# druskus20/volym

Hardware: AMD Instinct MI355X
Metric: Mrays/s + achieved HBM GB/s, 256^3 uint8 @ 1920x1080 (higher is better)
Workload: dtype u8 voxels, f32 compositing

## Files before the change

include/volym_hip.h:

```cpp
#ifndef VOLYM_HIP_H
#define VOLYM_HIP_H

#include <stddef.h>
#include <stdint.h>

#ifdef __cplusplus
extern "C" {
#endif

#define VOLYM_ABI_VERSION 2

enum {
    VOLYM_OK = 0,
    VOLYM_E_INVALID = -1,
    VOLYM_E_HIP = -2,
    VOLYM_E_NO_DEVICE = -3,
    VOLYM_E_NOMEM = -4,
    VOLYM_E_STATE = -5
};

enum { VOLYM_FILTER_NEAREST = 0, VOLYM_FILTER_LINEAR = 1 };

enum {
    VOLYM_OPT_KERNEL = 1,
// ... 9 lines not shown
    VOLYM_OPT_SETUP_IEEE = 10
};

typedef struct volym_camera_uniforms {
    float view_matrix[4][4];
    float projection_matrix[4][4];
    float inverse_view_proj[4][4];
    float camera_position[3];
    float _padding;
} volym_camera_uniforms;

typedef struct volym_parameter_uniforms {
    float density_threshold;
    uint32_t use_cone_importance_check;
    uint32_t use_importance_coloring;
    uint32_t use_opacity;
    uint32_t use_importance_rendering;
    uint32_t use_gaussian_smoothing;
    uint32_t importance_check_ahead_steps;
    float raymarching_step_size;
} volym_parameter_uniforms;

typedef struct volym_stats {
    uint64_t n_vol;
    uint64_t n_imp;
    uint64_t n_steps;
    uint64_t n_dense;
    uint64_t n_hit;
    uint64_t n_rays;
} volym_stats;

typedef struct volym_ctx volym_ctx;

int volym_create(volym_ctx** out, uint32_t width, uint32_t height, int device_id);
void volym_destroy(volym_ctx* ctx);
const char* volym_last_error(const volym_ctx* ctx);
int volym_abi_version(void);

int volym_set_stream(volym_ctx* ctx, void* hip_stream);
int volym_set_option(volym_ctx* ctx, int key, int value);

int volym_set_shard(volym_ctx* ctx, uint32_t rank, uint32_t world);

int volym_set_volume(volym_ctx* ctx, const uint8_t* voxels, uint32_t nx, uint32_t ny,
                     uint32_t nz, int filter);
int volym_set_importances(volym_ctx* ctx, const uint8_t* importances, uint32_t nx,
                          uint32_t ny, uint32_t nz);
int volym_set_labels(volym_ctx* ctx, const uint8_t* labels, uint32_t nx, uint32_t ny, uint32_t nz);
int volym_set_segment_importances(volym_ctx* ctx, const uint8_t table[256]);
int volym_label_counts(volym_ctx* ctx, uint64_t counts[256]);
int volym_set_transfer_function(volym_ctx* ctx, const uint8_t* rgba8, uint32_t n);

int volym_update(volym_ctx* ctx, const volym_camera_uniforms* camera,
                 const volym_parameter_uniforms* parameters);
int volym_compute_pass(volym_ctx* ctx);
int volym_sync(volym_ctx* ctx);
int volym_throttle(volym_ctx* ctx, uint32_t max_in_flight);
int volym_settle(volym_ctx* ctx);

int volym_read_rgba8(volym_ctx* ctx, uint8_t* out);
int volym_read_rgba32f(volym_ctx* ctx, float* out);

int volym_blit(volym_ctx* ctx, void* target_rgba8, uint32_t out_w, uint32_t out_h);
int volym_read_blit(volym_ctx* ctx, uint8_t* out);

uint32_t volym_local_tiles(const volym_ctx* ctx);
size_t volym_shard_bytes(const volym_ctx* ctx);
void* volym_shard_device_ptr(volym_ctx* ctx);
void* volym_frame_device_ptr(volym_ctx* ctx);
int volym_bind_output(volym_ctx* ctx, void* shard_rgba8, void* frame_rgba8);
int volym_assemble(volym_ctx* ctx, const void* gathered);
size_t volym_packed_shard_bytes(const volym_ctx* ctx, uint32_t tiles);
int volym_pack_shard(volym_ctx* ctx, void* packed_device, size_t capacity_bytes);
int volym_packed_tiles(volym_ctx* ctx, uint32_t* tiles_used, uint32_t* overflowed);
int volym_assemble_packed(volym_ctx* ctx, const void* gathered_device, size_t stride_bytes);
int volym_read_shard(volym_ctx* ctx, uint8_t* out);
int volym_assemble_host(volym_ctx* ctx, const uint8_t* gathered_host);

int volym_stats_pass(volym_ctx* ctx, volym_stats* out);
int volym_time_passes(volym_ctx* ctx, uint32_t n, float* ms_each);
int volym_time_batch(volym_ctx* ctx, uint32_t n, float* ms_total);
int volym_selftest_ray_setup(volym_ctx* ctx, unsigned long long out[3]);

#ifdef __cplusplus
}
#endif
#endif
```

volym_amd/_lib.py:

```python
import ctypes as C
import os

_HERE = os.path.dirname(os.path.abspath(__file__))
LIB_PATH = os.environ.get("VOLYM_HIP_LIB") or os.path.join(_HERE, "libvolym_hip.so")

OK, E_INVALID, E_HIP, E_NO_DEVICE, E_NOMEM, E_STATE = 0, -1, -2, -3, -4, -5
FILTER_NEAREST, FILTER_LINEAR = 0, 1
OPT_KERNEL, OPT_WRITE_F32, OPT_MACRO_CELLS = 1, 2, 3
OPT_VOLUME_LAYOUT, OPT_CULLING, OPT_COST_FEEDBACK, OPT_DEPTH_PARALLEL, OPT_XCD_BANDS, OPT_REBALANCE_ROUNDS = 4, 5, 6, 7, 8, 9
OPT_SETUP_IEEE = 10
OPT_FRAMES_IN_FLIGHT = 11


class VolymError(RuntimeError):
    def __init__(self, code, msg):
        super().__init__("volym error %d: %s" % (code, msg))
        self.code = code


class CameraUniforms(C.Structure):
    _fields_ = [
        ("view_matrix", (C.c_float * 4) * 4),
        ("projection_matrix", (C.c_float * 4) * 4),
        ("inverse_view_proj", (C.c_float * 4) * 4),
# ... 36 lines not shown
        ("distance", C.c_float),
        ("max_distance", C.c_float),
        ("min_distance", C.c_float),
    ]


class CCameraController(C.Structure):
    _fields_ = [(n, C.c_float) for n in
                ("rotate_horizontal", "rotate_vertical", "scroll", "sensitivity", "zoom_sensitivity")]


class CStateParameters(C.Structure):
    _fields_ = [
        ("camera_position", C.c_float * 3),
        ("density_trheshold", C.c_float),
        ("use_cone_importance_check", C.c_uint32),
        ("use_importance_coloring", C.c_uint32),
        ("use_opacity", C.c_uint32),
        ("use_importance_rendering", C.c_uint32),
        ("use_gaussian_smoothing", C.c_uint32),
        ("importance_check_ahead_steps", C.c_uint32),
        ("raymarching_step_size", C.c_float),
    ]


class CState(C.Structure):
    _fields_ = [
        ("camera", CCamera),
        ("camera_controller", CCameraController),
        ("density_threshold", C.c_float),
        ("use_importance_coloring", C.c_uint32),
        ("use_cone_importance_check", C.c_uint32),
        ("use_opacity", C.c_uint32),
        ("use_importance_rendering", C.c_uint32),
        ("use_gaussian_smoothing", C.c_uint32),
        ("importance_check_ahead_steps", C.c_uint32),
        ("raymarching_step_size", C.c_float),
    ]


_u8p = C.POINTER(C.c_uint8)
_f32p = C.POINTER(C.c_float)
_ctx = C.c_void_p

SIGNATURES = {
    "volym_create": (C.c_int, [C.POINTER(_ctx), C.c_uint32, C.c_uint32, C.c_int]),
    "volym_destroy": (None, [_ctx]),
    "volym_last_error": (C.c_char_p, [_ctx]),
    "volym_abi_version": (C.c_int, []),
    "volym_set_stream": (C.c_int, [_ctx, C.c_void_p]),
    "volym_set_option": (C.c_int, [_ctx, C.c_int, C.c_int]),
    "volym_set_shard": (C.c_int, [_ctx, C.c_uint32, C.c_uint32]),
    "volym_set_volume": (C.c_int, [_ctx, _u8p, C.c_uint32, C.c_uint32, C.c_uint32, C.c_int]),
    "volym_set_importances": (C.c_int, [_ctx, _u8p, C.c_uint32, C.c_uint32, C.c_uint32]),
    "volym_set_transfer_function": (C.c_int, [_ctx, _u8p, C.c_uint32]),
    "volym_set_labels": (C.c_int, [_ctx, _u8p, C.c_uint32, C.c_uint32, C.c_uint32]),
    "volym_set_segment_importances": (C.c_int, [_ctx, _u8p]),
    "volym_label_counts": (C.c_int, [_ctx, C.POINTER(C.c_uint64)]),
    "volym_update": (C.c_int, [_ctx, C.POINTER(CameraUniforms), C.POINTER(ParameterUniforms)]),
    "volym_compute_pass": (C.c_int, [_ctx]),
    "volym_sync": (C.c_int, [_ctx]),
    "volym_settle": (C.c_int, [_ctx]),
    "volym_throttle": (C.c_int, [_ctx, C.c_uint32]),
    "volym_blit": (C.c_int, [_ctx, C.c_void_p, C.c_uint32, C.c_uint32]),
    "volym_read_blit": (C.c_int, [_ctx, _u8p]),
    "volym_read_rgba8": (C.c_int, [_ctx, _u8p]),
    "volym_read_rgba32f": (C.c_int, [_ctx, _f32p]),
    "volym_local_tiles": (C.c_uint32, [_ctx]),
    "volym_shard_bytes": (C.c_size_t, [_ctx]),
    "volym_shard_device_ptr": (C.c_void_p, [_ctx]),
    "volym_frame_device_ptr": (C.c_void_p, [_ctx]),
    "volym_bind_output": (C.c_int, [_ctx, C.c_void_p, C.c_void_p]),
    "volym_assemble": (C.c_int, [_ctx, C.c_void_p]),
    "volym_packed_shard_bytes": (C.c_size_t, [_ctx, C.c_uint32]),
    "volym_pack_shard": (C.c_int, [_ctx, C.c_void_p, C.c_size_t]),
    "volym_packed_tiles": (C.c_int, [_ctx, C.POINTER(C.c_uint32), C.POINTER(C.c_uint32)]),
    "volym_assemble_packed": (C.c_int, [_ctx, C.c_void_p, C.c_size_t]),
    "volym_read_shard": (C.c_int, [_ctx, _u8p]),
    "volym_assemble_host": (C.c_int, [_ctx, _u8p]),
    "volym_stats_pass": (C.c_int, [_ctx, C.POINTER(Stats)]),
    "volym_time_passes": (C.c_int, [_ctx, C.c_uint32, _f32p]),
    "volym_time_batch": (C.c_int, [_ctx, C.c_uint32, _f32p]),
    "volym_selftest_ray_setup": (C.c_int, [_ctx, C.POINTER(C.c_ulonglong)]),
    "volym_camera_default_with_aspect_and_pos": (None, [C.POINTER(CCamera), C.c_float, _f32p]),
    "volym_camera_orbit": (None, [C.POINTER(CCamera), C.c_float, C.c_float, C.c_float]),
    "volym_camera_view_matrix": (None, [C.POINTER(CCamera), _f32p]),
    "volym_camera_projection_matrix": (None, [C.POINTER(CCamera), _f32p]),
    "volym_camera_uniforms_from": (C.c_int, [C.POINTER(CCamera), C.POINTER(CameraUniforms)]),
    "volym_camera_controller_new": (None, [C.POINTER(CCameraController), C.c_float, C.c_float]),
    "volym_camera_controller_process_mouse": (None, [C.POINTER(CCameraController), C.c_double, C.c_double]),
    "volym_camera_controller_process_scroll": (None, [C.POINTER(CCameraController), C.c_float]),
    "volym_camera_controller_update_camera": (None, [C.POINTER(CCameraController), C.POINTER(CCamera)]),
    "volym_state_parameters_default": (None, [C.POINTER(CStateParameters)]),
    "volym_state_parameters_benchmark": (None, [C.POINTER(CStateParameters)]),
    "volym_state_with_parameters": (None, [C.POINTER(CState), C.c_float, C.POINTER(CStateParameters)]),
    "volym_state_update": (None, [C.POINTER(CState)]),
    "volym_parameter_uniforms_from": (C.c_int, [C.POINTER(CState), C.POINTER(ParameterUniforms)]),
    "volym_transfer_function_default_lut": (None, [_u8p]),
    "volym_transfer_function_bake": (C.c_int, [_f32p, C.c_uint32, _f32p, C.c_uint32, _u8p]),
    "volym_prepare_volume": (C.c_int, [_u8p, C.c_size_t, C.c_uint32, C.c_uint32, C.c_uint32, C.c_int, _u8p]),
    "volym_map_segments_to_importance": (C.c_int, [_u8p, C.c_size_t, _u8p, _u8p, C.c_uint32]),
    "volym_synth_bonsai": (C.c_int, [C.c_uint32, C.c_uint32, _u8p, _u8p]),
    "volym_synth_teapot": (C.c_int, [C.c_uint32, C.c_uint32, C.c_uint32, C.c_uint32, _u8p, _u8p]),
}

_lib = None


def lib():
    global _lib
    if _lib is None:
        if not os.path.exists(LIB_PATH):
            raise ImportError(
                "%s is missing: build it with `python -c 'import __graft_entry__ as g; g.build()'` "
                "or `make -C volym_amd/csrc` (hipcc --offload-arch=gfx950)" % LIB_PATH)
        L = C.CDLL(LIB_PATH)
        for name, (res, args) in SIGNATURES.items():
            fn = getattr(L, name)
            fn.restype = res
            fn.argtypes = args
        _lib = L
    return _lib


def check(rc, ctx=None):
    if rc != OK:
        msg = lib().volym_last_error(ctx)
        raise VolymError(rc, msg.decode() if msg else "")
    return rc
```

volym_amd/csrc/context.hpp:

```cpp
#pragma once

#include <hip/hip_runtime.h>

#include <atomic>
#include <condition_variable>
#include <cstdint>
#include <memory>
#include <mutex>
#include <string>
#include <thread>
#include <vector>

#include "../../include/volym_hip.h"
#include "raymarch_device.h"

namespace volym {

struct WorkList {
    std::vector<uint32_t> entries;
    uint32_t grid = 0;
    uint64_t view_serial = 0;
    bool has_dp = false;
    bool trimmable = false;
    uint32_t trim_round = 0;
    bool final_for_view = false;
    std::vector<uint16_t> shares;
};

}

namespace volym {

struct FbJob {
    int list = 0;
    uint32_t n_entries = 0;
    uint64_t view_serial = 0;
    bool captured_has_dp = false;
    bool continuous = false;
    bool plain = false;
    uint32_t max_grid = 0, waves = 16;
    int dp_min_cost = -1;
    uint32_t dp_share_pct = 60, fill_cost = 2;
    bool super_fill = true, only_quarters = false;
    int dilate = -1;
    uint32_t grid = 0;
    uint32_t dev_drop_tenths = 0;
    uint32_t dp_floor = 64;
    uint32_t trim_rounds = 0;
    double t_us[6] = {};
    uint32_t prio_tenths[3] = {3, 6, 10};
    std::string error;
};

struct FrameSlot {
    hipStream_t stream = nullptr;
    hipStream_t own_stream = nullptr;
    hipStream_t copy_stream = nullptr;

    static constexpr int TABLE_RING = 8;
    FrameTables* d_tables = nullptr;
    FrameTables* h_tables[TABLE_RING] = {};
    hipEvent_t tables_ev[TABLE_RING] = {};
    int tables_slot = 0;
    FrameTables tables_now;
    bool tables_dirty = true;
    float tables_alpha_y = -1.0f;

    uint8_t* d_df = nullptr;
    uint32_t df_thr_byte = 0xffffffffu;
    uint32_t thr_byte_cull = 256;
    bool hull_dirty = true;
    uint32_t* d_tile_mask = nullptr;
    int mask_cur = 0;
    bool mask_wanted = false;
    bool mask_pending = false;
    uint32_t view_launches = 0;
    float mask_clip[16] = {};
    float mask_margin = 0.0f;
    uint32_t* d_tile_depth = nullptr;
    int* d_aabb = nullptr;

    uint32_t* d_shard_own = nullptr;
    uint32_t* d_frame_own = nullptr;
    float4* d_f32 = nullptr;
    uint32_t* d_blit = nullptr;
    size_t blit_bytes = 0;
    uint32_t blit_w = 0, blit_h = 0;
    uint8_t* d_gather_tmp = nullptr;
    uint32_t* d_pack_counters = nullptr;
    uint32_t pack_parity = 0;
    size_t gather_tmp_bytes = 0;
    Counters* d_counters = nullptr;
    uint4* d_trace = nullptr;

    uint32_t* d_list[2] = {nullptr, nullptr};
    uint32_t* h_list_pinned = nullptr;
    uint16_t* d_cost = nullptr;
    uint16_t* h_cost_pinned = nullptr;
    size_t list_capacity = 0;
    int cur = 0;
    WorkList lists[2];
    std::vector<uint16_t> item_cost;
    std::vector<uint8_t> item_is_dp;
    std::atomic<uint64_t> view_serial{1};
    uint32_t* d_pool_sync = nullptr;
    bool pool_launched = false;
    uint32_t* d_pool_dbg = nullptr;
    bool pool_dbg = false;

    enum : int { FB_IDLE = 0, FB_CAPTURED = 1, FB_READY = 2, FB_QUIT = 3 };
    std::thread fb_thread;
    std::mutex fb_mu;
    std::condition_variable fb_cv;
    std::atomic<int> fb_state{FB_IDLE};
    hipEvent_t ev_march = nullptr, ev_cost = nullptr, ev_list = nullptr;
    FbJob fb_job;

    FrameParams fp;
};

}

struct volym_ctx {
    int device = 0;
    uint32_t W = 0, H = 0, tiles_x = 0, tiles_y = 0, n_tiles = 0;
    uint32_t rank = 0, world = 1, n_local = 0, shard_tiles = 0;
    std::vector<uint32_t> geometric;

    uint8_t* d_vol = nullptr;
    uint8_t* d_imp = nullptr;
    uint32_t nx = 0, ny = 0, nz = 0;
    uint32_t inx = 0, iny = 0, inz = 0;
    int imp_box_lo[3] = {1, 1, 1}, imp_box_hi[3] = {0, 0, 0};
    uint64_t imp_bytes = 0;
    uint8_t* d_labels = nullptr;
    uint32_t lnx = 0, lny = 0, lnz = 0;
    bool labels_bricked = false;
    uint64_t label_count[256] = {};
    int label_box[256][6] = {};
    int filter = VOLYM_FILTER_NEAREST;
    uint8_t lut[256 * 4] = {};
    uint32_t tf_n = 0;
    bool have_vol = false, have_imp = false, have_tf = false, have_frame = false;

    uint8_t* d_mc = nullptr;
    std::vector<uint8_t> h_mc;
    int aabb_tab[257][6];
    uint32_t mc_n = 32;
    uint32_t tile_mask_words = 0;
    bool tile_mask = true;
    bool tile_depth = true;
    bool mask_eager = false;

    uint32_t* bound_shard = nullptr;
    uint32_t* bound_frame = nullptr;

    static constexpr uint32_t THROTTLE_RING = 9;
    hipEvent_t throttle_ev[THROTTLE_RING] = {};
    uint32_t throttle_head = 0;

    bool feedback = true;
    bool feedback_frozen = false;
    int wide_waves = 0;
    uint32_t trim_rounds = 0;
    int cost_dilate = -1;
    bool super_fill = true;
    uint32_t prio_tenths[3] = {3, 6, 10};
    bool dev_only_quarters = false;
    uint32_t dev_drop_tenths = 0;
    uint32_t dp_floor = 64;
    bool bricked = false;
    uint64_t brick_from_bytes = 64ull << 20;
    int layout_choice = -1;
    uint32_t dp_share_pct = 60;
    uint32_t fill_cost = 2;
    int dp_min_cost = -1;
    int n_cus = 256;
    uint32_t wgs_per_cu = 1;
    bool culling = true;
    bool setup_ieee = false;
    bool straight_jobs = false;
    bool lds_bricks = false;
    volym_camera_uniforms cam_copy;
    volym_parameter_uniforms par_copy;
    int kernel_variant = 2;
    bool write_f32 = false;
    uint32_t xcd_bands = 0;

    std::unique_ptr<volym::FrameSlot> slots[2];
    int last = 0;
    int last_blit = 0;
    uint32_t flight_parity = 0;
    std::string err;

    int n_slots() const { return slots[1] ? 2 : 1; }
    volym::FrameSlot& slot0() { return *slots[0]; }
    uint32_t* frame_buf(const volym::FrameSlot& s) const { return bound_frame ? bound_frame : s.d_frame_own; }
    uint32_t* shard_buf(const volym::FrameSlot& s) const { return bound_shard ? bound_shard : s.d_shard_own; }
};

namespace volym {

int ctx_fail(volym_ctx* c, int code, const std::string& msg);
int ctx_launch_march(volym_ctx* c);

}

#define VOLYM_HIPCHK(ctx, expr)                                                                          \
    do {                                                                                                 \
        hipError_t e_ = (expr);                                                                          \
        if (e_ != hipSuccess)                                                                            \
            return volym::ctx_fail(ctx, VOLYM_E_HIP, std::string(#expr) + ": " + hipGetErrorString(e_)); \
    } while (0)
```

volym_amd/csrc/raymarch.hip:

```cpp
#include <hip/hip_runtime.h>

#include <algorithm>
#include <cmath>
#include <cstdio>
#include <chrono>
#include <cstring>
#include <queue>
#include <string>
#include <vector>

#include "context.hpp"
#include "raymarch_kernels.h"
#include "raymarch_pq.h"
#include "raymarch_pool.h"
#include "blit.h"

namespace volym {
extern template __global__ void volym_raymarch_pq_kernel<true, false, false, 4, false, false, false, PQ_WAVES, 0, false>(
    const uint8_t* __restrict__, const uint8_t* __restrict__, const FrameTables* __restrict__, const uint8_t* __restrict__, const uint2* __restrict__, uint32_t,
    uint16_t* __restrict__, uint32_t* __restrict__, uint32_t* __restrict__, float4* __restrict__, Counters* __restrict__, uint4* __restrict__, const FrameParams);
}

using namespace volym;

static_assert(sizeof(volym_camera_uniforms) == 208, "CameraUniforms is 208 bytes (src/gpu_resources/camera.rs:56-64)");
static_assert(sizeof(volym_parameter_uniforms) == 32, "ParameterUniforms is 32 bytes (src/gpu_resources/parameters.rs:55-66)");

static const float k_cone_cos[8] = {0x1p+0f, 0x1.6a09f6p-1f, 0x1.54442ep-20f, -0x1.6a09bap-1f,
                                    -0x1p+0f, -0x1.6a0a32p-1f, -0x1.fe6644p-19f, 0x1.6a097ep-1f};
static const float k_cone_sin[8] = {0x0p+0f, 0x1.6a09d8p-1f, 0x1p+0f, 0x1.6a0a14p-1f,
                                    0x1.54442ep-19f, -0x1.6a099cp-1f, -0x1p+0f, -0x1.6a0a5p-1f};

static thread_local std::string g_create_error;

int volym::ctx_fail(volym_ctx* c, int code, const std::string& msg)
{
    if (c) c->err = msg; else g_create_error = msg;
    return code;
}
static int fail(volym_ctx* c, int code, const std::string& msg) { return ctx_fail(c, code, msg); }
#define HIPCHK(ctx, expr) VOLYM_HIPCHK(ctx, expr)

static void recompute_shard(volym_ctx* c)
{
    c->n_local = c->n_tiles > c->rank ? (c->n_tiles - c->rank + c->world - 1) / c->world : 0;
    c->shard_tiles = (c->n_tiles + c->world - 1) / c->world;
}

static uint32_t max_grid(const volym_ctx* c) { return static_cast<uint32_t>(c->n_cus) * c->wgs_per_cu; }

static bool frame_uses_pool(const volym_ctx* c, uint32_t flags)
{
    return c->kernel_variant == 3 && !(flags & (F_LINEAR | F_GAUSSIAN | F_IMP_COLORING | F_IMP_RENDERING)) && (flags & F_OPACITY);
}

static void host_texel_linear(float u, int n, int& i0, int& i1, float& w)
{
    const float x = u * static_cast<float>(n) - 0.5f;
    float fl = std::floor(x);
    w = x - fl;
    if (!(fl >= -2.0f)) fl = -2.0f;
    if (fl > static_cast<float>(n)) fl = static_cast<float>(n);
    const int i = static_cast<int>(fl);
    i0 = i < 0 ? 0 : (i > n - 1 ? n - 1 : i);
    i1 = i + 1 < 0 ? 0 : (i + 1 > n - 1 ? n - 1 : i + 1);
}

static void build_tables(volym_ctx* c, FrameTables& t, float alpha_y)
{
    const int n = static_cast<int>(c->tf_n);
    for (int b = 0; b < 256; ++b) {
        t.rho[b] = static_cast<float>(b) / 255.0f;
        const uint8_t* q = c->lut + 4 * (b < n ? b : n - 1);
        t.lut_f[b] = make_float4(static_cast<float>(q[0]) / 255.0f, static_cast<float>(q[1]) / 255.0f,
                                 static_cast<float>(q[2]) / 255.0f, static_cast<float>(q[3]) / 255.0f);
    }
    for (int b = 0; b < 256; ++b) {
        int i0, i1;
        float w;
        host_texel_linear(t.rho[b], n, i0, i1, w);
        const float4 a = t.lut_f[i0], bb = t.lut_f[i1];
        const float iw = 1.0f - w;
        const float A = a.w * iw + bb.w * w;
        t.tf_tab[b] = make_float4(a.x * iw + bb.x * w, a.y * iw + bb.y * w, a.z * iw + bb.z * w,
                                  1.0f - wgsl_pow(1.0f - A, alpha_y));
        t.ic_alpha[b] = 1.0f - wgsl_pow(1.0f - t.rho[b], alpha_y);
    }
}
namespace {
struct P2 { double x, y; };

bool invert4d(const double m[16], double inv[16])
{
    double a[4][8];
    for (int r = 0; r < 4; ++r)
        for (int col = 0; col < 4; ++col) { a[r][col] = m[col * 4 + r]; a[r][4 + col] = r == col ? 1.0 : 0.0; }
    for (int i = 0; i < 4; ++i) {
        int piv = i;
        for (int r = i + 1; r < 4; ++r) if (std::fabs(a[r][i]) > std::fabs(a[piv][i])) piv = r;
        if (std::fabs(a[piv][i]) < 1e-300) return false;
        if (piv != i) for (int k = 0; k < 8; ++k) std::swap(a[i][k], a[piv][k]);
// ... 516 lines not shown
    c->have_vol = true;
    c->have_frame = had_frame;
    return VOLYM_OK;
}

static void set_reject_box(const volym_ctx* c, FrameParams& fp)
{
    const uint32_t dims[3] = {c->inx, c->iny, c->inz};
    for (int a = 0; a < 3; ++a) {
        if (c->imp_box_lo[a] > c->imp_box_hi[a]) { fp.imp_lo[a] = INFINITY; fp.imp_hi[a] = -INFINITY; continue; }
        fp.imp_lo[a] = c->imp_box_lo[a] <= 0 ? -INFINITY : static_cast<float>(c->imp_box_lo[a]) / static_cast<float>(dims[a]) - 2.0e-6f;
        fp.imp_hi[a] = c->imp_box_hi[a] >= static_cast<int>(dims[a]) - 1 ? INFINITY : static_cast<float>(c->imp_box_hi[a] + 1) / static_cast<float>(dims[a]) + 2.0e-6f;
    }
}

extern "C" {

int volym_abi_version(void) { return VOLYM_ABI_VERSION; }

const char* volym_last_error(const volym_ctx* ctx) { return ctx ? ctx->err.c_str() : g_create_error.c_str(); }


static int init_slot(volym_ctx* c, FrameSlot& s)
{
    auto bad = [&](hipError_t e, const char* what) {
        return fail(c, e == hipErrorOutOfMemory ? VOLYM_E_NOMEM : VOLYM_E_HIP, std::string(what) + ": " + hipGetErrorString(e));
    };
    HIPCHK(c, hipSetDevice(c->device));
    std::memset(&s.fp, 0, sizeof s.fp);
    std::memset(&s.tables_now, 0, sizeof s.tables_now);
    hipError_t e;
    if ((e = hipStreamCreateWithFlags(&s.own_stream, hipStreamNonBlocking)) != hipSuccess) return bad(e, "hipStreamCreate");
    if ((e = hipStreamCreateWithFlags(&s.copy_stream, hipStreamNonBlocking)) != hipSuccess) return bad(e, "hipStreamCreate");
    s.stream = s.own_stream;
    const size_t frame_bytes = static_cast<size_t>(c->W) * c->H * 4;
    if ((e = hipMalloc(&s.d_frame_own, frame_bytes)) != hipSuccess) return bad(e, "hipMalloc(frame)");
    if ((e = hipMalloc(&s.d_shard_own, static_cast<size_t>(c->n_tiles) * 1024)) != hipSuccess) return bad(e, "hipMalloc(shard)");
    if ((e = hipMalloc(&s.d_tables, sizeof(FrameTables))) != hipSuccess) return bad(e, "hipMalloc(tables)");
    if ((e = hipMalloc(&s.d_counters, sizeof(Counters))) != hipSuccess) return bad(e, "hipMalloc(counters)");
    if ((e = hipMemset(s.d_frame_own, 0, frame_bytes)) != hipSuccess) return bad(e, "hipMemset(frame)");
    if ((e = hipMalloc(&s.d_aabb, 6 * sizeof(int))) != hipSuccess) return bad(e, "hipMalloc(aabb)");
    if (c->tile_mask_words && (e = hipMalloc(&s.d_tile_mask, 2u * c->tile_mask_words * sizeof(uint32_t))) != hipSuccess) return bad(e, "hipMalloc(tile mask)");
    if (c->tile_mask_words && (e = hipMemset(s.d_tile_mask, 0, 2u * c->tile_mask_words * sizeof(uint32_t))) != hipSuccess) return bad(e, "hipMemset(tile mask)");
    if (c->tile_mask_words && (e = hipMalloc(&s.d_tile_depth, 64u * static_cast<size_t>(c->tile_mask_words) * sizeof(uint32_t))) != hipSuccess) return bad(e, "hipMalloc(tile depth)");
    if ((e = hipMalloc(&s.d_pack_counters, 4 * sizeof(uint32_t))) != hipSuccess) return bad(e, "hipMalloc(pack counters)");
    if ((e = hipMemset(s.d_pack_counters, 0, 4 * sizeof(uint32_t))) != hipSuccess) return bad(e, "hipMemset(pack counters)");
    if ((e = hipMalloc(&s.d_pool_sync, 4 * sizeof(uint32_t))) != hipSuccess) return bad(e, "hipMalloc(pool sync)");
    if ((e = hipMemset(s.d_pool_sync, 0, 4 * sizeof(uint32_t))) != hipSuccess) return bad(e, "hipMemset(pool sync)");
    if ((e = hipMalloc(&s.d_pool_dbg, static_cast<size_t>(c->n_cus) * 8u * PL_WAVES * 24u * sizeof(uint32_t))) != hipSuccess) return bad(e, "hipMalloc(pool timeline)");
    for (int i = 0; i < FrameSlot::TABLE_RING; ++i) {
        if ((e = hipHostMalloc(reinterpret_cast<void**>(&s.h_tables[i]), sizeof(FrameTables), hipHostMallocDefault)) != hipSuccess) return bad(e, "hipHostMalloc(tables)");
        if ((e = hipEventCreateWithFlags(&s.tables_ev[i], hipEventDisableTiming)) != hipSuccess) return bad(e, "hipEventCreate");
    }
    if ((e = hipEventCreateWithFlags(&s.ev_march, hipEventDisableTiming)) != hipSuccess) return bad(e, "hipEventCreate");
    if ((e = hipEventCreateWithFlags(&s.ev_cost, hipEventDisableTiming)) != hipSuccess) return bad(e, "hipEventCreate");
    if ((e = hipEventCreateWithFlags(&s.ev_list, hipEventDisableTiming)) != hipSuccess) return bad(e, "hipEventCreate");
    if (c->write_f32 && (e = hipMalloc(&s.d_f32, static_cast<size_t>(c->W) * c->H * sizeof(float4))) != hipSuccess) return bad(e, "hipMalloc(f32 frame)");
    const int rc = reset_slot_lists(c, s);
    if (rc != VOLYM_OK) return rc;
    try {
        s.fb_thread = std::thread(feedback_thread, c, &s);
    } catch (...) {
        return fail(c, VOLYM_E_NOMEM, "cannot start the feedback thread");
    }
    return VOLYM_OK;
}

static void free_slot(FrameSlot& s)
{
    if (s.fb_thread.joinable()) {
        feedback_quiesce(s);
        {
            std::lock_guard<std::mutex> lk(s.fb_mu);
            s.fb_state.store(FrameSlot::FB_QUIT, std::memory_order_release);
        }
        s.fb_cv.notify_all();
        s.fb_thread.join();
    }
    if (s.stream) (void)hipStreamSynchronize(s.stream);
    if (s.copy_stream) (void)hipStreamSynchronize(s.copy_stream);
    (void)hipFree(s.d_tables); (void)hipFree(s.d_df);
    (void)hipFree(s.d_shard_own); (void)hipFree(s.d_frame_own); (void)hipFree(s.d_f32); (void)hipFree(s.d_blit);
    (void)hipFree(s.d_gather_tmp); (void)hipFree(s.d_pack_counters); (void)hipFree(s.d_counters); (void)hipFree(s.d_aabb); (void)hipFree(s.d_tile_mask);
    (void)hipFree(s.d_tile_depth);
    (void)hipFree(s.d_list[0]); (void)hipFree(s.d_list[1]); (void)hipFree(s.d_cost);
    (void)hipFree(s.d_pool_sync); (void)hipFree(s.d_pool_dbg);
    if (s.h_list_pinned) (void)hipHostFree(s.h_list_pinned);
    if (s.h_cost_pinned) (void)hipHostFree(s.h_cost_pinned);
    for (int i = 0; i < FrameSlot::TABLE_RING; ++i) {
        if (s.h_tables[i]) (void)hipHostFree(s.h_tables[i]);
        if (s.tables_ev[i]) (void)hipEventDestroy(s.tables_ev[i]);
    }
    if (s.ev_march) (void)hipEventDestroy(s.ev_march);
    if (s.ev_cost) (void)hipEventDestroy(s.ev_cost);
    if (s.ev_list) (void)hipEventDestroy(s.ev_list);
    if (s.own_stream) (void)hipStreamDestroy(s.own_stream);
    if (s.copy_stream) (void)hipStreamDestroy(s.copy_stream);
}

static int refuse_two_slots(volym_ctx* c, const char* what)
{
    return fail(c, VOLYM_E_STATE, std::string(what) + ": not with VOLYM_OPT_FRAMES_IN_FLIGHT = 2");
}

int volym_create(volym_ctx** out, uint32_t width, uint32_t height, int device_id)
{
    if (!out) return fail(nullptr, VOLYM_E_INVALID, "volym_create: out is NULL");
    *out = nullptr;
    if (width == 0 || height == 0 || width > 32768 || height > 32768)
        return fail(nullptr, VOLYM_E_INVALID, "volym_create: viewport must be 1..32768 in each dimension");
    int n_dev = 0;
    if (hipGetDeviceCount(&n_dev) != hipSuccess || n_dev <= 0)
        return fail(nullptr, VOLYM_E_NO_DEVICE, "volym_create: no HIP device visible");
    int dev = device_id;
    if (dev < 0) { if (hipGetDevice(&dev) != hipSuccess) dev = 0; }
    if (dev >= n_dev) return fail(nullptr, VOLYM_E_NO_DEVICE, "volym_create: device_id out of range");
    hipDeviceProp_t prop;
    HIPCHK(nullptr, hipGetDeviceProperties(&prop, dev));
    if (std::strncmp(prop.gcnArchName, "gfx950", 6) != 0)
        return fail(nullptr, VOLYM_E_NO_DEVICE,
                    std::string("volym_create: this library carries gfx950 code only, device is ") + prop.gcnArchName);
    HIPCHK(nullptr, hipSetDevice(dev));

    volym_ctx* c = new (std::nothrow) volym_ctx();
    if (!c) return fail(nullptr, VOLYM_E_NOMEM, "volym_create: out of host memory");
    c->device = dev;
    c->n_cus = prop.multiProcessorCount > 0 ? prop.multiProcessorCount : 256;
    c->W = width; c->H = height;
    c->tiles_x = (width + 15u) / 16u;
    c->tiles_y = (height + 15u) / 16u;
    c->n_tiles = c->tiles_x * c->tiles_y;
    recompute_shard(c);
    std::memset(c->aabb_tab, 0, sizeof c->aabb_tab);
    const uint64_t tiles8 = static_cast<uint64_t>(c->tiles_x) * 2u * c->tiles_y * 2u;
    const uint64_t words = (tiles8 + 31u) / 32u;
    c->tile_mask_words = words <= VOLYM_TILE_MASK_MAX_WORDS ? static_cast<uint32_t>(words) : 0u;
    build_geometric(c);

    c->slots[0].reset(new (std::nothrow) FrameSlot());
    const int rc = c->slots[0] ? init_slot(c, c->slot0()) : fail(c, VOLYM_E_NOMEM, "out of host memory");
    if (rc != VOLYM_OK) { const std::string m = c->err; volym_destroy(c); return fail(nullptr, rc, m); }
    *out = c;
    return VOLYM_OK;
}

void volym_destroy(volym_ctx* c)
{
    if (!c) return;
    (void)hipSetDevice(c->device);
    for (int i = 1; i >= 0; --i)
        if (c->slots[i]) free_slot(*c->slots[i]);
    (void)hipFree(c->d_vol); (void)hipFree(c->d_imp); (void)hipFree(c->d_labels); (void)hipFree(c->d_mc);
    for (uint32_t i = 0; i < volym_ctx::THROTTLE_RING; ++i) if (c->throttle_ev[i]) (void)hipEventDestroy(c->throttle_ev[i]);
    delete c;
}

int volym_set_stream(volym_ctx* c, void* hip_stream)
{
    if (!c) return VOLYM_E_INVALID;
    if (c->slots[1]) return refuse_two_slots(c, "volym_set_stream");
    FrameSlot& s = c->slot0();
    HIPCHK(c, hipSetDevice(c->device));
    feedback_quiesce(s);
    HIPCHK(c, hipStreamSynchronize(s.stream));
    s.stream = hip_stream ? static_cast<hipStream_t>(hip_stream) : s.own_stream;
    return VOLYM_OK;
}
// ... 52 lines not shown
            if (e != hipSuccess) { c->write_f32 = false; return fail(c, VOLYM_E_NOMEM, std::string("hipMalloc(f32 frame): ") + hipGetErrorString(e)); }
        }
        return VOLYM_OK;
    case VOLYM_OPT_MACRO_CELLS:
        if (value < 4 || value > (VOLYM_DEV_SWITCHES ? 64 : 32) || (value & (value - 1)) != 0)
            return fail(c, VOLYM_E_INVALID, "VOLYM_OPT_MACRO_CELLS: power of two in 4..32");
        c->mc_n = static_cast<uint32_t>(value);
        if (c->have_vol) { int rc = build_macro_cells(c); if (rc != VOLYM_OK) return rc; }
        return rebuild_lists(c);
    case VOLYM_OPT_VOLUME_LAYOUT:
        if (value < -1 || value > 1) return fail(c, VOLYM_E_INVALID, "VOLYM_OPT_VOLUME_LAYOUT: -1 (by size), 0 (linear) or 1 (4x4x4 bricks)");
        c->layout_choice = value;
        return VOLYM_OK;
    case VOLYM_OPT_CULLING:
        c->culling = value != 0;
        for (int i = 0; i < c->n_slots(); ++i) c->slots[i]->hull_dirty = true;
        return VOLYM_OK;
    case VOLYM_OPT_COST_FEEDBACK:
        c->feedback = value != 0;
        return rebuild_lists(c);
    case VOLYM_OPT_DEPTH_PARALLEL:
        if (value < -100 || value > 65535) return fail(c, VOLYM_E_INVALID, "VOLYM_OPT_DEPTH_PARALLEL: < 0 adaptive (-N = N/10 x fair share), 0 off, else explicit cost");
        c->dp_min_cost = value;
        return rebuild_lists(c);
    case VOLYM_OPT_REBALANCE_ROUNDS:
        if (value < 0 || value > 8) return fail(c, VOLYM_E_INVALID, "VOLYM_OPT_REBALANCE_ROUNDS: 0..8");
        c->trim_rounds = static_cast<uint32_t>(value);
        return VOLYM_OK;
    case VOLYM_OPT_SETUP_IEEE:
        if (value != 0 && value != 1) return fail(c, VOLYM_E_INVALID, "VOLYM_OPT_SETUP_IEEE: 0 or 1");
        c->setup_ieee = value == 1;
        return VOLYM_OK;
    case VOLYM_OPT_XCD_BANDS:
        if (value < 0 || value > 64) return fail(c, VOLYM_E_INVALID, "VOLYM_OPT_XCD_BANDS: 0..64");
        c->xcd_bands = static_cast<uint32_t>(value);
        return VOLYM_OK;
#if VOLYM_DEV_SWITCHES
    case 101:
        if (value < 1 || value > 8) return fail(c, VOLYM_E_INVALID, "workgroups per CU: 1..8");
        c->wgs_per_cu = static_cast<uint32_t>(value);
        return rebuild_lists(c);
    case 107:
        c->super_fill = value != 0;
        return rebuild_lists(c);
    case 108:
        if (value < 0) return fail(c, VOLYM_E_INVALID, "priority thresholds: t1 + 100*t2 + 10000*t3, tenths of the fair share");
        c->prio_tenths[0] = static_cast<uint32_t>(value % 100);
        c->prio_tenths[1] = static_cast<uint32_t>((value / 100) % 100);
        c->prio_tenths[2] = static_cast<uint32_t>(value / 10000);
        return rebuild_lists(c);
    case 109:
        c->dev_only_quarters = value != 0;
        return rebuild_lists(c);
    case 110:
        for (int i = 0; i < c->n_slots(); ++i) c->slots[i]->fp.dev = static_cast<uint32_t>(value);
        return VOLYM_OK;
    case 113:
        for (int i = 0; i < c->n_slots(); ++i) feedback_quiesce(*c->slots[i]);
        c->feedback_frozen = value != 0;
        return VOLYM_OK;
    case 114:
        c->cost_dilate = std::max(-1, std::min(value, 4));
        return VOLYM_OK;
    case 115:
        if (value != 0 && value != 12 && value != 16) return fail(c, VOLYM_E_INVALID, "wide waves: 0, 12 or 16");
        c->wide_waves = value;
        return rebuild_lists(c);
    case 119:
        c->dp_floor = static_cast<uint32_t>(std::max(value, 1));
        return rebuild_lists(c);
    case 118:
        c->dev_drop_tenths = static_cast<uint32_t>(std::max(value, 0));
        return rebuild_lists(c);
    case 121:
        c->straight_jobs = value != 0;
        return VOLYM_OK;
    case 122:
        c->lds_bricks = value != 0;
        return VOLYM_OK;
    case 123:
        c->tile_depth = value != 0;
        for (int i = 0; i < c->n_slots(); ++i) c->slots[i]->hull_dirty = true;
        return rebuild_lists(c);
    case 117:
        c->tile_mask = value != 0;
        c->mask_eager = value == 2;
        for (int i = 0; i < c->n_slots(); ++i) c->slots[i]->hull_dirty = true;
        return rebuild_lists(c);
    case 111:
        c->dp_share_pct = static_cast<uint32_t>(value % 1000);
        c->fill_cost = static_cast<uint32_t>(value / 1000);
        return rebuild_lists(c);
#endif
    default:
        return fail(c, VOLYM_E_INVALID, "volym_set_option: unknown key");
    }
}

int volym_set_shard(volym_ctx* c, uint32_t rank, uint32_t world)
{
    if (!c) return VOLYM_E_INVALID;
    if (world == 0 || rank >= world || world > 4096) return fail(c, VOLYM_E_INVALID, "volym_set_shard: need rank < world <= 4096");
    const int rc = quiesce_slots(c);
    if (rc != VOLYM_OK) return rc;
    c->rank = rank; c->world = world;
    recompute_shard(c);
    return rebuild_lists(c);
}

static uint64_t layout_bytes(bool bricked, uint32_t nx, uint32_t ny, uint32_t nz)
{
    return bricked ? static_cast<uint64_t>(brick_count(nx)) * brick_count(ny) * brick_count(nz) * 64u : static_cast<uint64_t>(nx) * ny * nz;
}

static int upload_volume(volym_ctx* c, uint8_t** dst, const uint8_t* src, uint32_t nx, uint32_t ny, uint32_t nz)
{
    const bool bricked = want_bricked(c, nx, ny, nz);
    if (!src || nx == 0 || ny == 0 || nz == 0) return fail(c, VOLYM_E_INVALID, "volume: NULL data or zero dimension");
    const uint64_t n = static_cast<uint64_t>(nx) * ny * nz;
    const uint64_t nb = layout_bytes(bricked, nx, ny, nz);
    if (nx > 4096 || ny > 4096 || nz > 4096 || nb > 0xffffffffull)
        return fail(c, VOLYM_E_INVALID, "volume: each dimension <= 4096 and the brick-padded size < 2^32");
    const int rc = quiesce_slots(c);
    if (rc != VOLYM_OK) return rc;
    if (*dst) { HIPCHK(c, hipFree(*dst)); *dst = nullptr; }
    uint8_t* staging = nullptr;
    hipError_t e = hipMalloc(dst, nb + 16);
    if (e == hipSuccess) e = hipMemset(*dst + nb, 0, 16);
    if (e == hipSuccess && bricked) e = hipMalloc(&staging, n);
    if (e != hipSuccess) { (void)hipFree(staging); return fail(c, VOLYM_E_NOMEM, std::string("hipMalloc(volume): ") + hipGetErrorString(e)); }
    e = hipMemcpy(bricked ? staging : *dst, src, n, hipMemcpyHostToDevice);
    if (e == hipSuccess && bricked) {
        const hipStream_t stream = c->slot0().stream;
        hipLaunchKernelGGL(volym_rebrick_kernel, dim3(static_cast<uint32_t>((nb + 255u) / 256u)), dim3(256), 0, stream, staging, *dst, nx, ny, nz);
        e = hipGetLastError();
        if (e == hipSuccess) e = hipStreamSynchronize(stream);
    }
    (void)hipFree(staging);
    if (e != hipSuccess) return fail(c, VOLYM_E_HIP, std::string("volume upload: ") + hipGetErrorString(e));
    return VOLYM_OK;
}

static bool want_bricked(const volym_ctx* c, uint32_t nx, uint32_t ny, uint32_t nz)
{
    if (c->layout_choice >= 0) return c->layout_choice == 1;
    return static_cast<uint64_t>(nx) * ny * nz > c->brick_from_bytes;
}

int volym_set_volume(volym_ctx* c, const uint8_t* voxels, uint32_t nx, uint32_t ny, uint32_t nz, int filter)
{
    if (!c) return VOLYM_E_INVALID;
    if (filter != VOLYM_FILTER_NEAREST && filter != VOLYM_FILTER_LINEAR)
        return fail(c, VOLYM_E_INVALID, "volym_set_volume: filter must be VOLYM_FILTER_NEAREST or VOLYM_FILTER_LINEAR");
    int rc = upload_volume(c, &c->d_vol, voxels, nx, ny, nz);
    if (rc != VOLYM_OK) { c->have_vol = false; return rc; }
    c->nx = nx; c->ny = ny; c->nz = nz; c->filter = filter;
    c->bricked = want_bricked(c, nx, ny, nz);
    rc = build_macro_cells(c);
    if (rc != VOLYM_OK) { c->have_vol = false; return rc; }
    return rebuild_lists(c);
}

static void important_texel_box(const uint8_t* imp, uint32_t nx, uint32_t ny, uint32_t nz, int (&lo)[3], int (&hi)[3])
{
    int x0 = INT32_MAX, y0 = INT32_MAX, z0 = INT32_MAX, x1 = -1, y1 = -1, z1 = -1;
    for (uint32_t z = 0; z < nz; ++z)
        for (uint32_t y = 0; y < ny; ++y) {
            const uint8_t* row = imp + (static_cast<size_t>(z) * ny + y) * nx;
            int first = -1, last = -1;
            uint32_t x = 0;
            for (; x + 8u <= nx; x += 8u) {
                uint64_t w;
                std::memcpy(&w, row + x, 8);
                w &= 0x8080808080808080ull;
                if (!w) continue;
                if (first < 0) first = static_cast<int>(x) + (__builtin_ctzll(w) >> 3);
                last = static_cast<int>(x) + 7 - (__builtin_clzll(w) >> 3);
            }
            for (; x < nx; ++x)
                if (row[x] & 0x80u) { if (first < 0) first = static_cast<int>(x); last = static_cast<int>(x); }
            if (first < 0) continue;
            x0 = std::min(x0, first); x1 = std::max(x1, last);
            y0 = std::min(y0, static_cast<int>(y)); y1 = std::max(y1, static_cast<int>(y));
            z0 = std::min(z0, static_cast<int>(z)); z1 = std::max(z1, static_cast<int>(z));
        }
    if (x1 < 0) { lo[0] = lo[1] = lo[2] = 1; hi[0] = hi[1] = hi[2] = 0; return; }
    lo[0] = x0; lo[1] = y0; lo[2] = z0; hi[0] = x1; hi[1] = y1; hi[2] = z1;
}

// ... 34 lines not shown
    hipError_t e = hipMalloc(&d_stats, init.size());
    if (e == hipSuccess) e = hipMemcpy(d_stats, init.data(), init.size(), hipMemcpyHostToDevice);
    if (e == hipSuccess) {
        hipLaunchKernelGGL(volym_label_stats_kernel, dim3(stream_grid(c, n_chunks)), dim3(256), 0, stream, reinterpret_cast<const uint4*>(c->d_labels),
                           reinterpret_cast<unsigned long long*>(d_stats), reinterpret_cast<int*>(d_stats + 256 * sizeof(unsigned long long)),
                           nx, ny, nz, c->labels_bricked ? 1u : 0u, static_cast<uint32_t>(n_chunks));
        e = hipGetLastError();
    }
    if (e == hipSuccess) e = hipMemcpyAsync(init.data(), d_stats, init.size(), hipMemcpyDeviceToHost, stream);
    if (e == hipSuccess) e = hipStreamSynchronize(stream);
    (void)hipFree(d_stats);
    if (e != hipSuccess) {
        (void)hipFree(c->d_labels); c->d_labels = nullptr;
        return fail(c, VOLYM_E_HIP, std::string("volym_set_labels: ") + hipGetErrorString(e));
    }
    std::memcpy(c->label_count, init.data(), sizeof c->label_count);
    std::memcpy(c->label_box, boxes, sizeof c->label_box);
    return VOLYM_OK;
}

int volym_set_segment_importances(volym_ctx* c, const uint8_t table[256])
{
    if (!c) return VOLYM_E_INVALID;
    if (!table) return fail(c, VOLYM_E_INVALID, "volym_set_segment_importances: NULL table");
    if (!c->d_labels) return fail(c, VOLYM_E_STATE, "volym_set_segment_importances: no labels (volym_set_labels first; volym_set_importances drops them)");
    int rc = quiesce_slots(c);
    if (rc != VOLYM_OK) return rc;
    const uint64_t nb = layout_bytes(c->labels_bricked, c->lnx, c->lny, c->lnz);
    if (c->imp_bytes != nb + 16u) {
        c->have_imp = false;
        if (c->d_imp) { HIPCHK(c, hipFree(c->d_imp)); c->d_imp = nullptr; }
        c->imp_bytes = 0;
        hipError_t e = hipMalloc(&c->d_imp, nb + 16u);
        if (e == hipSuccess) e = hipMemset(c->d_imp + nb, 0, 16);
        if (e != hipSuccess) { (void)hipFree(c->d_imp); c->d_imp = nullptr; return fail(c, VOLYM_E_NOMEM, std::string("hipMalloc(importances): ") + hipGetErrorString(e)); }
        c->imp_bytes = nb + 16u;
    }
    LabelTable t;
    std::memcpy(t.v, table, 256);
    const uint64_t n_chunks = (nb + 15u) / 16u;
    const hipStream_t stream = c->slot0().stream;
    hipLaunchKernelGGL(volym_segment_map_kernel, dim3(stream_grid(c, n_chunks)), dim3(256), 0, stream, reinterpret_cast<const uint4*>(c->d_labels),
                       reinterpret_cast<uint4*>(c->d_imp), t, c->lnx, c->lny, c->lnz, c->labels_bricked ? 1u : 0u, static_cast<uint32_t>(n_chunks));
    HIPCHK(c, hipGetLastError());
    HIPCHK(c, hipStreamSynchronize(stream));
    int lo[3] = {INT32_MAX, INT32_MAX, INT32_MAX}, hi[3] = {-1, -1, -1};
    for (int l = 0; l < 256; ++l) {
        if (table[l] < 128u || c->label_count[l] == 0u) continue;
        for (int a = 0; a < 3; ++a) { lo[a] = std::min(lo[a], c->label_box[l][a]); hi[a] = std::max(hi[a], c->label_box[l][3 + a]); }
    }
    for (int a = 0; a < 3; ++a) {
        if (hi[0] < 0) { c->imp_box_lo[a] = 1; c->imp_box_hi[a] = 0; continue; }
        c->imp_box_lo[a] = lo[a]; c->imp_box_hi[a] = hi[a];
    }
    c->inx = c->lnx; c->iny = c->lny; c->inz = c->lnz;
    c->have_imp = true;
    for (int i = 0; i < c->n_slots(); ++i) set_reject_box(c, c->slots[i]->fp);
    return rebuild_lists(c);
}

int volym_label_counts(volym_ctx* c, uint64_t counts[256])
{
    if (!c) return VOLYM_E_INVALID;
    if (!counts) return fail(c, VOLYM_E_INVALID, "volym_label_counts: NULL output");
    if (!c->d_labels) return fail(c, VOLYM_E_STATE, "volym_label_counts: no labels");
    std::memcpy(counts, c->label_count, sizeof c->label_count);
    return VOLYM_OK;
}

int volym_set_transfer_function(volym_ctx* c, const uint8_t* rgba8, uint32_t n)
{
    if (!c) return VOLYM_E_INVALID;
    if (!rgba8 || n < 1 || n > 256) return fail(c, VOLYM_E_INVALID, "volym_set_transfer_function: 1..256 RGBA8 texels");
    std::memset(c->lut, 0, sizeof c->lut);
    std::memcpy(c->lut, rgba8, static_cast<size_t>(n) * 4);
    c->tf_n = n;
    c->have_tf = true;
    for (int i = 0; i < c->n_slots(); ++i) c->slots[i]->tables_dirty = true;
    return VOLYM_OK;
}

}

static int ensure_frame_resources(volym_ctx* c, FrameSlot& s)
{
    if (s.df_thr_byte != s.thr_byte_cull) {
        if (c->mc_n <= 32u) hipLaunchKernelGGL(volym_distance_field_kernel<1>, dim3(1), dim3(1024), 0, s.stream, c->d_mc, s.d_df, s.d_aabb, c->mc_n, s.thr_byte_cull);
        else hipLaunchKernelGGL(volym_distance_field_kernel<4>, dim3(1), dim3(1024), 0, s.stream, c->d_mc, s.d_df, s.d_aabb, c->mc_n, s.thr_byte_cull);
        HIPCHK(c, hipGetLastError());
        s.df_thr_byte = s.thr_byte_cull;
        s.hull_dirty = true;
    }
    if (s.hull_dirty) {
        compute_culling(c, s);
        s.fp.tile_mask = nullptr;
        s.fp.tile_depth = nullptr;
        s.fp.mask_words = c->tile_mask_words;
        s.fp.tile_mask_spare = s.d_tile_mask ? s.d_tile_mask + static_cast<size_t>(s.mask_cur ^ 1) * c->tile_mask_words : nullptr;
        s.mask_pending = s.mask_wanted;
        s.view_launches = 0;
    }
    if (s.mask_pending && (s.view_launches >= 1u || c->mask_eager)) {
        ClipMatrix M;
        std::memcpy(M.m, s.mask_clip, sizeof M.m);
        s.mask_cur ^= 1;
        uint32_t* cur = s.d_tile_mask + static_cast<size_t>(s.mask_cur) * c->tile_mask_words;
        const uint32_t cells = c->mc_n * c->mc_n * c->mc_n;
        if (static_cast<size_t>(c->tile_mask_words) * sizeof(uint32_t) <= 48u * 1024u) {
            const uint32_t nb = (c->mc_n + 7u) / 8u;
            hipLaunchKernelGGL(volym_tile_mask_lds_kernel, dim3(nb * nb * ((c->mc_n + 3u) / 4u)), dim3(256), c->tile_mask_words * sizeof(uint32_t), s.stream, c->d_mc, c->mc_n,
                               s.thr_byte_cull, M, s.mask_margin, c->W, c->H, c->tiles_x * 2u, c->tile_mask_words, cur);
        } else {
            hipLaunchKernelGGL(volym_tile_mask_kernel, dim3((cells + 255u) / 256u), dim3(256), 0, s.stream, c->d_mc, c->mc_n, s.thr_byte_cull, M, s.mask_margin,
                               c->W, c->H, c->tiles_x * 2u, c->tile_mask_words, cur);
        }
        HIPCHK(c, hipGetLastError());
        s.fp.tile_mask = cur;
        s.fp.cull |= CULL_TILE_MASK;
        if (c->tile_depth && s.d_tile_depth) {
            const uint32_t n_t8 = 32u * c->tile_mask_words;
            HIPCHK(c, hipMemsetAsync(s.d_tile_depth, 0, 2u * static_cast<size_t>(n_t8) * sizeof(uint32_t), s.stream));
            const uint32_t nb = (c->mc_n + 7u) / 8u;
            hipLaunchKernelGGL(volym_tile_depth_kernel, dim3(nb * nb * ((c->mc_n + 3u) / 4u)), dim3(256), 0, s.stream, c->d_mc, c->mc_n, s.thr_byte_cull, M,
                               s.mask_margin, s.fp.eye[0], s.fp.eye[1], s.fp.eye[2], c->W, c->H, c->tiles_x * 2u, n_t8, s.d_tile_depth);
            HIPCHK(c, hipGetLastError());
            s.fp.tile_depth = s.d_tile_depth;
            s.fp.cull |= CULL_TILE_DEPTH;
        }
        s.fp.tile_mask_spare = s.d_tile_mask + static_cast<size_t>(s.mask_cur ^ 1) * c->tile_mask_words;
        s.mask_pending = false;
        if (s.view_launches >= 1u) s.view_serial.fetch_add(1, std::memory_order_relaxed);
    }
    s.view_launches++;
    return VOLYM_OK;
}

static int update_slot(volym_ctx* c, FrameSlot& s, const volym_camera_uniforms* cam, const volym_parameter_uniforms* par, bool view_changed)
{
    const float step = par->raymarching_step_size;
    FrameParams& fp = s.fp;
    std::memcpy(fp.ivp, cam->inverse_view_proj, sizeof fp.ivp);
    fp.eye[0] = cam->camera_position[0]; fp.eye[1] = cam->camera_position[1]; fp.eye[2] = cam->camera_position[2];
    fp.thr = par->density_threshold;
    fp.base_step = step;
    fp.min_step = step * 0.25f;
    fp.alpha_y = fp.min_step * 100.0f;
    fp.flags = (par->use_cone_importance_check == 1u ? F_CONE : 0u) | (par->use_importance_coloring == 1u ? F_IMP_COLORING : 0u) |
               (par->use_opacity == 1u ? F_OPACITY : 0u) | (par->use_importance_rendering == 1u ? F_IMP_RENDERING : 0u) |
               (par->use_gaussian_smoothing == 1u ? F_GAUSSIAN : 0u) | (c->filter == VOLYM_FILTER_LINEAR ? F_LINEAR : 0u);
    fp.ahead_steps = par->importance_check_ahead_steps;
    fp.W = c->W; fp.H = c->H;
    {
        fp.rcp_w = static_cast<float>(1.0 / static_cast<double>(c->W));
        fp.rcp_h = static_cast<float>(1.0 / static_cast<double>(c->H));
        bool vouch = c->W <= 16384u && c->H <= 16384u && !c->setup_ieee;
        for (int i = 0; i < 16; ++i) vouch = vouch && std::fabs(fp.ivp[i]) < 0x1p+60f;
        for (int i = 0; i < 3; ++i) {
            const float n0 = std::fabs(0.0f - fp.eye[i]), n1 = std::fabs(1.0f - fp.eye[i]);
            vouch = vouch && n0 >= 0x1p-40f && n0 <= 0x1p+40f && n1 >= 0x1p-40f && n1 <= 0x1p+40f;
        }
        fp.setup_lo = vouch ? 0x1p-40f : INFINITY;
    }
    fp.nx = c->nx; fp.ny = c->ny; fp.nz = c->nz;
    fp.tiles_x = c->tiles_x; fp.n_tiles = c->n_tiles;
    fp.tf_n = c->tf_n;
    set_reject_box(c, fp);
    const float sigma = 1.5f;
    for (int i = -2; i <= 2; ++i) {
        const float x = static_cast<float>(i) * 0.005f;
        fp.gauss_w[i + 2] = wgsl_exp(-(x * x) / (2.0f * sigma * sigma));
    }
    std::memcpy(fp.cone_cos, k_cone_cos, sizeof k_cone_cos);
    std::memcpy(fp.cone_sin, k_cone_sin, sizeof k_cone_sin);

    if (s.tables_dirty || s.tables_alpha_y != fp.alpha_y) {
        const int slot = s.tables_slot;
        s.tables_slot = (slot + 1) % FrameSlot::TABLE_RING;
        if (hipEventQuery(s.tables_ev[slot]) != hipSuccess) HIPCHK(c, hipEventSynchronize(s.tables_ev[slot]));
        build_tables(c, *s.h_tables[slot], fp.alpha_y);
        s.tables_now = *s.h_tables[slot];
        HIPCHK(c, hipMemcpyAsync(s.d_tables, s.h_tables[slot], sizeof(FrameTables), hipMemcpyHostToDevice, s.stream));
        HIPCHK(c, hipEventRecord(s.tables_ev[slot], s.stream));
        s.tables_dirty = false;
        s.tables_alpha_y = fp.alpha_y;
    }
    uint32_t tb = 256;
    for (int b = 255; b >= 0; --b)
        if (s.tables_now.rho[b] >= fp.thr) tb = static_cast<uint32_t>(b); else break;
    fp.thr_byte = tb;
    if (fp.flags & (F_LINEAR | F_GAUSSIAN)) {
        const float cons = fp.thr - std::fabs(fp.thr) * 1.0e-5f - 1.0e-7f;
        uint32_t tc = 256;
        for (int b = 255; b >= 0; --b)
            if (s.tables_now.rho[b] >= cons) tc = static_cast<uint32_t>(b); else break;
        s.thr_byte_cull = tc;
    } else {
        s.thr_byte_cull = tb;
    }
    if (view_changed) {
        s.view_serial.fetch_add(1, std::memory_order_relaxed);
        s.hull_dirty = true;
    }
    return VOLYM_OK;
}

extern "C" {

int volym_update(volym_ctx* c, const volym_camera_uniforms* cam, const volym_parameter_uniforms* par)
{
    if (!c) return VOLYM_E_INVALID;
    if (!cam || !par) return fail(c, VOLYM_E_INVALID, "volym_update: NULL uniforms");
    if (!c->have_vol || !c->have_imp || !c->have_tf)
        return fail(c, VOLYM_E_STATE, "volym_update: set volume, importances and transfer function first");
    if (c->nx != c->inx || c->ny != c->iny || c->nz != c->inz)
        return fail(c, VOLYM_E_STATE, "volym_update: volume and importances differ in size");
    const float step = par->raymarching_step_size;
    if (!(step >= 1.0e-4f && step <= 1.0f)) return fail(c, VOLYM_E_INVALID, "volym_update: raymarching_step_size must be in [1e-4, 1]");
    if (!std::isfinite(par->density_threshold)) return fail(c, VOLYM_E_INVALID, "volym_update: density_threshold is not finite");
    if (par->importance_check_ahead_steps > 4096u) return fail(c, VOLYM_E_INVALID, "volym_update: importance_check_ahead_steps > 4096");
    for (int i = 0; i < 16; ++i)
        if (!std::isfinite((&cam->inverse_view_proj[0][0])[i])) return fail(c, VOLYM_E_INVALID, "volym_update: inverse_view_proj is not finite");
    for (int i = 0; i < 3; ++i)
        if (!(std::fabs(cam->camera_position[i]) <= 64.0f)) return fail(c, VOLYM_E_INVALID, "volym_update: |camera_position| must be <= 64 per axis");

    HIPCHK(c, hipSetDevice(c->device));
    const bool view_changed = !c->have_frame || std::memcmp(&c->cam_copy, cam, sizeof *cam) != 0 || std::memcmp(&c->par_copy, par, sizeof *par) != 0;
    for (int i = 0; i < c->n_slots(); ++i) {
        const int rc = update_slot(c, *c->slots[i], cam, par, view_changed);
        if (rc != VOLYM_OK) return rc;
    }
    c->cam_copy = *cam;
    c->par_copy = *par;
    c->have_frame = true;
    return VOLYM_OK;
}

}

template <bool COUNT, bool TRACE = false>
static int launch_march(volym_ctx* c, FrameSlot& s)
{
    int rc = ensure_frame_resources(c, s);
    if (rc != VOLYM_OK) return rc;
    FrameParams fp = s.fp;
    fp.rank = c->rank; fp.world = c->world; fp.n_local = c->n_local;
    fp.mc_n = c->mc_n;
    fp.xcd_bands = c->xcd_bands;
    if (c->world == 1) fp.flags |= F_RASTER;
    if (c->write_f32 && c->world == 1) fp.flags |= F_WRITE_F32;
    if (c->n_local == 0) return VOLYM_OK;
    uint32_t grid = c->n_local;
    if (fp.xcd_bands) {
        const uint32_t chunks = 8u * fp.xcd_bands;
        const uint32_t per_chunk = (c->n_local + chunks - 1u) / chunks;
        grid = per_chunk * chunks;
    }
    uint32_t* const d_shard = c->shard_buf(s);
    uint32_t* const d_frame = c->frame_buf(s);
    Counters* cnt = (COUNT || (VOLYM_DEV_SWITCHES && (s.fp.dev & 512u))) ? s.d_counters : nullptr;
    uint4* trace = TRACE ? s.d_trace : nullptr;
    if (!COUNT && !TRACE && frame_uses_pool(c, fp.flags)) {
        const uint32_t pgrid = std::min(256u, max_grid(c));
        uint32_t* dbg = s.pool_dbg ? s.d_pool_dbg : nullptr;
        if (c->bricked)
            hipLaunchKernelGGL((volym_raymarch_pool_kernel<true>), dim3(pgrid), dim3(PL_WAVES * 64), 0, s.stream, c->d_vol, s.d_tables, s.d_df, s.d_pool_sync, d_shard,
                               d_frame, s.d_f32, dbg, fp);
        else
            hipLaunchKernelGGL((volym_raymarch_pool_kernel<false>), dim3(pgrid), dim3(PL_WAVES * 64), 0, s.stream, c->d_vol, s.d_tables, s.d_df, s.d_pool_sync, d_shard,
                               d_frame, s.d_f32, dbg, fp);
        HIPCHK(c, hipGetLastError());
        s.pool_launched = true;
        return VOLYM_OK;
    }
    if (c->kernel_variant >= 2) {
        const bool plain = !COUNT && !TRACE;
        if (plain) feedback_poll(s);
        const WorkList& wl = s.lists[s.cur];
        const uint32_t n_items = static_cast<uint32_t>(wl.entries.size());
        if (n_items == 0) return VOLYM_OK;
        const bool capture = plain && c->feedback && !c->feedback_frozen && s.fb_state.load(std::memory_order_acquire) == FrameSlot::FB_IDLE && (wl.view_serial != s.view_serial.load(std::memory_order_relaxed) || !wl.final_for_view);
        uint16_t* cost_out = capture ? s.d_cost : nullptr;
        const bool table = !(fp.flags & (F_LINEAR | F_GAUSSIAN));
        const bool special = !COUNT && !(fp.flags & F_IMP_COLORING) && (fp.flags & F_OPACITY);
        const bool no_imp = special && !(fp.flags & F_IMP_RENDERING);
        const bool ir = special && (fp.flags & F_IMP_RENDERING);
        const bool wide12 = c->wide_waves == 12 || (c->wide_waves == 0 && c->bricked && ir);
        const uint32_t waves = ((table && no_imp) || !wide12) ? PQ_WAVES : PQ_WAVES_WIDE;
        const uint32_t want = (n_items + waves - 1) / waves;
        const uint32_t pgrid = wl.grid ? wl.grid : std::max(1u, std::min(want, max_grid(c)));
#define VOLYM_PQ_LAUNCH_J(T, KS, I, B, R, WV, J)                                                                                 \
    hipLaunchKernelGGL((volym_raymarch_pq_kernel<T, COUNT && I, TRACE, KS, I, B, R, WV, J>), dim3(pgrid), dim3(WV * 64), 0, s.stream, c->d_vol,  \
                       c->d_imp, s.d_tables, s.d_df, reinterpret_cast<const uint2*>(s.d_list[s.cur]), n_items, cost_out, d_shard, d_frame, s.d_f32, cnt, trace, fp)
#define VOLYM_PQ_LAUNCH(T, KS, I, B, R, WV) VOLYM_PQ_LAUNCH_J(T, KS, I, B, R, WV, 0)
#if VOLYM_DEV_SWITCHES
#define VOLYM_PQ_LAUNCH_W(T, KS, I, B, R) do { if (wide12) VOLYM_PQ_LAUNCH(T, KS, I, B, R, PQ_WAVES_WIDE); else VOLYM_PQ_LAUNCH(T, KS, I, B, R, PQ_WAVES); } while (0)
#else
#define VOLYM_PQ_LAUNCH_W(T, KS, I, B, R) VOLYM_PQ_LAUNCH(T, KS, I, B, R, PQ_WAVES)
#endif
        const bool cone_jobs = ir && (fp.flags & F_CONE) != 0u && !TRACE;
        const bool straight_jobs = VOLYM_DEV_SWITCHES && ir && !(fp.flags & F_CONE) && !TRACE && c->straight_jobs;
        (void)straight_jobs;
        if (c->bricked) {
#if VOLYM_DEV_SWITCHES
            if (table && no_imp && c->lds_bricks && !COUNT && !TRACE)
                hipLaunchKernelGGL((volym_raymarch_pq_kernel<true, false, false, 4, false, true, false, PQ_WAVES, 0, true>), dim3(pgrid), dim3(PQ_WAVES * 64), 0, s.stream, c->d_vol,
                                   c->d_imp, s.d_tables, s.d_df, reinterpret_cast<const uint2*>(s.d_list[s.cur]), n_items, cost_out, d_shard, d_frame, s.d_f32, cnt, trace, fp);
            else
#endif
            if (table && no_imp) VOLYM_PQ_LAUNCH(true, 4, false, true, false, PQ_WAVES);
            else if (table && ir && cone_jobs) VOLYM_PQ_LAUNCH_J(true, 4, false, true, true, PQ_WAVES, 1);
#if VOLYM_DEV_SWITCHES
            else if (table && ir && straight_jobs) VOLYM_PQ_LAUNCH_J(true, 4, false, true, true, PQ_WAVES, 2);
#endif
            else if (table && ir) { if (wide12) VOLYM_PQ_LAUNCH(true, 4, false, true, true, PQ_WAVES_WIDE); else VOLYM_PQ_LAUNCH(true, 4, false, true, true, PQ_WAVES); }
            else if (table) VOLYM_PQ_LAUNCH_W(true, 4, true, true, false);
            else VOLYM_PQ_LAUNCH_W(false, 1, true, true, false);
        } else {
            if (table && no_imp) VOLYM_PQ_LAUNCH(true, 4, false, false, false, PQ_WAVES);
            else if (table && ir && cone_jobs) VOLYM_PQ_LAUNCH_J(true, 4, false, false, true, PQ_WAVES, 1);
#if VOLYM_DEV_SWITCHES
            else if (table && ir && straight_jobs) VOLYM_PQ_LAUNCH_J(true, 4, false, false, true, PQ_WAVES, 2);
#endif
            else if (table && ir) VOLYM_PQ_LAUNCH_W(true, 4, false, false, true);
            else if (table) VOLYM_PQ_LAUNCH_W(true, 4, true, false, false);
            else VOLYM_PQ_LAUNCH_W(false, 1, true, false, false);
        }
#undef VOLYM_PQ_LAUNCH_W
#undef VOLYM_PQ_LAUNCH
#undef VOLYM_PQ_LAUNCH_J
        HIPCHK(c, hipGetLastError());
        if (capture) {
            HIPCHK(c, hipEventRecord(s.ev_march, s.stream));
            HIPCHK(c, hipStreamWaitEvent(s.copy_stream, s.ev_march, 0));
            const size_t cost_bytes = static_cast<size_t>((n_items + 1u) & ~1u) * sizeof(uint16_t) + static_cast<size_t>(pgrid) * (waves + 1u) * sizeof(uint32_t);
            HIPCHK(c, hipMemcpyAsync(s.h_cost_pinned, s.d_cost, cost_bytes, hipMemcpyDeviceToHost, s.copy_stream));
            HIPCHK(c, hipEventRecord(s.ev_cost, s.copy_stream));
            FbJob& job = s.fb_job;
            job.list = s.cur;
            job.n_entries = n_items;
            job.view_serial = s.view_serial.load(std::memory_order_relaxed);
            job.captured_has_dp = wl.has_dp;
            job.continuous = (fp.flags & (F_LINEAR | F_GAUSSIAN)) != 0u;
            job.plain = table && no_imp;
            job.max_grid = max_grid(c);
            job.waves = waves;
            job.dp_min_cost = c->dp_min_cost;
            job.dp_share_pct = c->dp_share_pct;
            job.fill_cost = c->fill_cost;
            job.super_fill = c->super_fill;
            job.only_quarters = c->dev_only_quarters;
            job.dilate = c->cost_dilate;
            job.grid = pgrid;
            job.dev_drop_tenths = c->dev_drop_tenths;
            job.dp_floor = c->dp_floor;
            job.trim_rounds = c->trim_rounds;
            job.t_us[0] = std::chrono::duration<double, std::micro>(std::chrono::steady_clock::now().time_since_epoch()).count();
            for (int i = 0; i < 3; ++i) job.prio_tenths[i] = c->prio_tenths[i];
            {
                std::lock_guard<std::mutex> lk(s.fb_mu);
                s.fb_state.store(FrameSlot::FB_CAPTURED, std::memory_order_release);
            }
            s.fb_cv.notify_all();
        }
        return VOLYM_OK;
    }
#define VOLYM_DIRECT_LAUNCH(V, B)                                                                                                \
    hipLaunchKernelGGL((volym_raymarch_kernel<V, COUNT, TRACE, B>), dim3(grid), dim3(256), 0, s.stream, c->d_vol, c->d_imp, s.d_tables, \
                       s.d_df, d_shard, d_frame, s.d_f32, cnt, trace, fp)
    if (c->kernel_variant >= 1) { if (c->bricked) VOLYM_DIRECT_LAUNCH(1, true); else VOLYM_DIRECT_LAUNCH(1, false); }
    else { if (c->bricked) VOLYM_DIRECT_LAUNCH(0, true); else VOLYM_DIRECT_LAUNCH(0, false); }
#undef VOLYM_DIRECT_LAUNCH
    HIPCHK(c, hipGetLastError());
    return VOLYM_OK;
}

int volym::ctx_launch_march(volym_ctx* c) { return launch_march<false>(c, c->slot0()); }

extern "C" {

int volym_compute_pass(volym_ctx* c)
{
    if (!c) return VOLYM_E_INVALID;
    if (!c->have_frame) return fail(c, VOLYM_E_STATE, "volym_compute_pass: call volym_update first");
    HIPCHK(c, hipSetDevice(c->device));
    c->last = c->slots[1] ? static_cast<int>(c->flight_parity++ & 1u) : 0;
    return launch_march<false>(c, *c->slots[c->last]);
}

int volym_throttle(volym_ctx* c, uint32_t max_in_flight)
{
    if (!c) return VOLYM_E_INVALID;
    if (max_in_flight == 0 || max_in_flight >= volym_ctx::THROTTLE_RING) return fail(c, VOLYM_E_INVALID, "volym_throttle: max_in_flight must be 1..8");
    HIPCHK(c, hipSetDevice(c->device));
    const uint32_t slot = c->throttle_head % volym_ctx::THROTTLE_RING;
    if (!c->throttle_ev[slot] && hipEventCreateWithFlags(&c->throttle_ev[slot], hipEventDisableTiming | hipEventDisableSystemFence) != hipSuccess) {
        (void)hipGetLastError();
        c->throttle_ev[slot] = nullptr;
        HIPCHK(c, hipEventCreateWithFlags(&c->throttle_ev[slot], hipEventDisableTiming));
    }
    HIPCHK(c, hipEventRecord(c->throttle_ev[slot], c->slots[c->last]->stream));
    c->throttle_head++;
    if (c->throttle_head > max_in_flight) {
        const uint32_t old = (c->throttle_head - 1u - max_in_flight) % volym_ctx::THROTTLE_RING;
        if (c->throttle_ev[old]) HIPCHK(c, hipEventSynchronize(c->throttle_ev[old]));
    }
    return VOLYM_OK;
}

static int check_pool_error(volym_ctx* c, FrameSlot& s)
{
    if (!s.pool_launched) return VOLYM_OK;
    uint32_t bits = 0;
// ... 145 lines not shown
}

int volym_packed_tiles(volym_ctx* c, uint32_t* tiles_used, uint32_t* overflowed)
{
    if (c && c->slots[1]) return refuse_two_slots(c, "volym_packed_tiles");
    if (!c || !tiles_used) return VOLYM_E_INVALID;
    FrameSlot& s = c->slot0();
    HIPCHK(c, hipSetDevice(c->device));
    uint32_t h[4] = {0, 0, 0, 0};
    HIPCHK(c, hipMemcpyAsync(h, s.d_pack_counters, sizeof(h), hipMemcpyDeviceToHost, s.stream));
    HIPCHK(c, hipStreamSynchronize(s.stream));
    *tiles_used = h[s.pack_parity ^ 1u];
    if (overflowed) *overflowed = h[2];
    return VOLYM_OK;
}

int volym_assemble_packed(volym_ctx* c, const void* gathered, size_t stride_bytes)
{
    if (c && c->slots[1]) return refuse_two_slots(c, "volym_assemble_packed");
    if (!c || !gathered) return VOLYM_E_INVALID;
    FrameSlot& s = c->slot0();
    if (stride_bytes < pack_header_bytes(c->shard_tiles)) return fail(c, VOLYM_E_INVALID, "volym_assemble_packed: stride smaller than the header");
    HIPCHK(c, hipSetDevice(c->device));
    hipLaunchKernelGGL(volym_assemble_packed_kernel, dim3(c->n_tiles), dim3(256), 0, s.stream, static_cast<const uint8_t*>(gathered), stride_bytes,
                       c->frame_buf(s), c->W, c->H, c->tiles_x, c->n_tiles, c->world, c->shard_tiles);
    HIPCHK(c, hipGetLastError());
    return VOLYM_OK;
}

int volym_assemble(volym_ctx* c, const void* gathered)
{
    if (c && c->slots[1]) return refuse_two_slots(c, "volym_assemble");
    if (!c || !gathered) return VOLYM_E_INVALID;
    FrameSlot& s = c->slot0();
    HIPCHK(c, hipSetDevice(c->device));
    hipLaunchKernelGGL(volym_assemble_kernel, dim3(c->n_tiles), dim3(256), 0, s.stream, static_cast<const uint32_t*>(gathered),
                       c->frame_buf(s), c->W, c->H, c->tiles_x, c->n_tiles, c->world, c->shard_tiles);
    HIPCHK(c, hipGetLastError());
    return VOLYM_OK;
}

int volym_assemble_host(volym_ctx* c, const uint8_t* gathered_host)
{
    if (c && c->slots[1]) return refuse_two_slots(c, "volym_assemble_host");
    if (!c || !gathered_host) return VOLYM_E_INVALID;
    FrameSlot& s = c->slot0();
    HIPCHK(c, hipSetDevice(c->device));
    const size_t bytes = volym_shard_bytes(c) * c->world;
    if (s.gather_tmp_bytes < bytes) {
        HIPCHK(c, hipStreamSynchronize(s.stream));
        if (s.d_gather_tmp) { HIPCHK(c, hipFree(s.d_gather_tmp)); s.d_gather_tmp = nullptr; s.gather_tmp_bytes = 0; }
        hipError_t e = hipMalloc(&s.d_gather_tmp, bytes);
        if (e != hipSuccess) return fail(c, VOLYM_E_NOMEM, std::string("hipMalloc(gather): ") + hipGetErrorString(e));
        s.gather_tmp_bytes = bytes;
    }
    HIPCHK(c, hipMemcpyAsync(s.d_gather_tmp, gathered_host, bytes, hipMemcpyHostToDevice, s.stream));
    HIPCHK(c, hipStreamSynchronize(s.stream));
    return volym_assemble(c, s.d_gather_tmp);
}

int volym_stats_pass(volym_ctx* c, volym_stats* out)
{
    if (!c || !out) return VOLYM_E_INVALID;
    FrameSlot& s = c->slot0();
    if (!c->have_frame) return fail(c, VOLYM_E_STATE, "volym_stats_pass: call volym_update first");
    HIPCHK(c, hipSetDevice(c->device));
    HIPCHK(c, hipMemsetAsync(s.d_counters, 0, sizeof(Counters), s.stream));
    int rc = launch_march<true>(c, s);
    if (rc != VOLYM_OK) return rc;
    Counters h;
    HIPCHK(c, hipMemcpyAsync(&h, s.d_counters, sizeof h, hipMemcpyDeviceToHost, s.stream));
    HIPCHK(c, hipStreamSynchronize(s.stream));
    out->n_vol = h.n_vol; out->n_imp = h.n_imp; out->n_steps = h.n_steps; out->n_dense = h.n_dense; out->n_hit = h.n_hit;
    uint64_t rays = 0;
    for (uint32_t k = c->rank; k < c->n_tiles; k += c->world) {
        const uint32_t tx = k % c->tiles_x, ty = k / c->tiles_x;
        const uint32_t w = std::min(16u, c->W - tx * 16u), h2 = std::min(16u, c->H - ty * 16u);
        rays += static_cast<uint64_t>(w) * h2;
    }
    out->n_rays = rays;
    return VOLYM_OK;
}

int volym_selftest_ray_setup(volym_ctx* c, unsigned long long out[3])
{
    if (!c || !out) return VOLYM_E_INVALID;
    FrameSlot& s = c->slot0();
    if (!c->have_frame) return fail(c, VOLYM_E_STATE, "volym_selftest_ray_setup: call volym_update first");
    HIPCHK(c, hipSetDevice(c->device));
    static_assert(sizeof(Counters) >= 3 * sizeof(unsigned long long), "counters");
    HIPCHK(c, hipMemsetAsync(s.d_counters, 0, sizeof(Counters), s.stream));
    const dim3 grid((c->W + 63u) / 64u, (c->H + 3u) / 4u);
    volym_ray_setup_selftest_kernel<<<grid, 256, 0, s.stream>>>(s.fp, reinterpret_cast<unsigned long long*>(s.d_counters));
    HIPCHK(c, hipGetLastError());
    Counters h;
    HIPCHK(c, hipMemcpyAsync(&h, s.d_counters, sizeof h, hipMemcpyDeviceToHost, s.stream));
    HIPCHK(c, hipStreamSynchronize(s.stream));
    out[0] = h.n_vol; out[1] = h.n_imp; out[2] = h.n_steps;
    return VOLYM_OK;
}

int volym_time_batch(volym_ctx* c, uint32_t n, float* ms_total)
{
    if (!c || !ms_total || n == 0 || n > 1000000) return VOLYM_E_INVALID;
    FrameSlot& s = c->slot0();
    if (!c->have_frame) return fail(c, VOLYM_E_STATE, "volym_time_batch: call volym_update first");
    HIPCHK(c, hipSetDevice(c->device));
    hipEvent_t e0 = nullptr, e1 = nullptr;
    if (hipEventCreate(&e0) != hipSuccess || hipEventCreate(&e1) != hipSuccess) { if (e0) (void)hipEventDestroy(e0); return fail(c, VOLYM_E_HIP, "hipEventCreate failed"); }
    int rc = ensure_frame_resources(c, s);
    if (rc == VOLYM_OK) {
        (void)hipEventRecord(e0, s.stream);
        for (uint32_t i = 0; i < n && rc == VOLYM_OK; ++i) rc = launch_march<false>(c, s);
        (void)hipEventRecord(e1, s.stream);
        if (hipStreamSynchronize(s.stream) != hipSuccess && rc == VOLYM_OK) rc = fail(c, VOLYM_E_HIP, "hipStreamSynchronize failed");
        if (rc == VOLYM_OK && hipEventElapsedTime(ms_total, e0, e1) != hipSuccess) rc = fail(c, VOLYM_E_HIP, "hipEventElapsedTime failed");
    }
    (void)hipEventDestroy(e0); (void)hipEventDestroy(e1);
    return rc;
}

int volym_time_passes(volym_ctx* c, uint32_t n, float* ms_each)
{
    if (!c || !ms_each || n == 0 || n > 100000) return VOLYM_E_INVALID;
    FrameSlot& s = c->slot0();
    if (!c->have_frame) return fail(c, VOLYM_E_STATE, "volym_time_passes: call volym_update first");
    HIPCHK(c, hipSetDevice(c->device));
    std::vector<hipEvent_t> ev(n + 1, nullptr);
    int rc = VOLYM_OK;
    for (uint32_t i = 0; i <= n && rc == VOLYM_OK; ++i)
        if (hipEventCreate(&ev[i]) != hipSuccess) rc = fail(c, VOLYM_E_HIP, "hipEventCreate failed");
    if (rc == VOLYM_OK) rc = ensure_frame_resources(c, s);
    if (rc == VOLYM_OK) {
        (void)hipEventRecord(ev[0], s.stream);
        for (uint32_t i = 0; i < n && rc == VOLYM_OK; ++i) {
            rc = launch_march<false>(c, s);
            if (hipEventRecord(ev[i + 1], s.stream) != hipSuccess && rc == VOLYM_OK) rc = fail(c, VOLYM_E_HIP, "hipEventRecord failed");
        }
        if (hipStreamSynchronize(s.stream) != hipSuccess && rc == VOLYM_OK) rc = fail(c, VOLYM_E_HIP, "hipStreamSynchronize failed");
        if (rc == VOLYM_OK)
            for (uint32_t i = 0; i < n; ++i)
                if (hipEventElapsedTime(&ms_each[i], ev[i], ev[i + 1]) != hipSuccess) { rc = fail(c, VOLYM_E_HIP, "hipEventElapsedTime failed"); break; }
    }
    for (auto e : ev) if (e) (void)hipEventDestroy(e);
    return rc;
}

#if VOLYM_DEV_SWITCHES
int volym_dev_pool_timeline(volym_ctx* c, int on, uint32_t* out, uint32_t max_words)
{
    if (!c) return VOLYM_E_INVALID;
    FrameSlot& s = c->slot0();
    HIPCHK(c, hipSetDevice(c->device));
    HIPCHK(c, hipStreamSynchronize(s.stream));
    const uint32_t words = std::min(max_words, static_cast<uint32_t>(max_grid(c)) * PL_WAVES * 24u);
    if (out && words) HIPCHK(c, hipMemcpy(out, s.d_pool_dbg, static_cast<size_t>(words) * sizeof(uint32_t), hipMemcpyDeviceToHost));
    s.pool_dbg = on != 0;
    return static_cast<int>(words);
}

int volym_dev_counters(volym_ctx* c, unsigned long long out[5], int reset)
{
    if (!c) return VOLYM_E_INVALID;
    FrameSlot& s = c->slot0();
    HIPCHK(c, hipSetDevice(c->device));
    HIPCHK(c, hipStreamSynchronize(s.stream));
// ... 71 lines not shown
```

volym_amd/csrc/raymarch_common.hip:

```cpp
#include <hip/hip_runtime.h>

#include "raymarch_pq.h"

namespace volym {

template __global__ void volym_raymarch_pq_kernel<true, false, false, 4, false, false, false, PQ_WAVES, 0, false>(
    const uint8_t* __restrict__, const uint8_t* __restrict__, const FrameTables* __restrict__, const uint8_t* __restrict__, const uint2* __restrict__, uint32_t,
    uint16_t* __restrict__, uint32_t* __restrict__, uint32_t* __restrict__, float4* __restrict__, Counters* __restrict__, uint4* __restrict__, const FrameParams);

}
```

volym_amd/csrc/raymarch_device.h:

```cpp
#pragma once

#include <hip/hip_runtime.h>

#include "wgsl_math.h"

namespace volym {

enum : uint32_t {
    F_CONE = 1u << 0,
    F_IMP_COLORING = 1u << 1,
    F_OPACITY = 1u << 2,
    F_IMP_RENDERING = 1u << 3,
    F_GAUSSIAN = 1u << 4,
    F_LINEAR = 1u << 5,
    F_WRITE_F32 = 1u << 6,
    F_RASTER = 1u << 7,
};

struct FrameParams {
    float ivp[16];
    float eye[3];
    float thr;
    float base_step;
    float min_step;
    float alpha_y;
    uint32_t flags;
    uint32_t ahead_steps;
    uint32_t W, H;
    uint32_t nx, ny, nz;
    uint32_t tiles_x, n_tiles;
    uint32_t rank, world, n_local;
    uint32_t thr_byte;
    uint32_t tf_n;
    uint32_t mc_n;
    uint32_t xcd_bands;
    float gauss_w[5];
    float cone_cos[8], cone_sin[8];
    uint32_t cull;
    float hull[2][8][4];
    float aabb_lo[3], aabb_hi[3];
    float imp_lo[3], imp_hi[3];
    uint32_t dev;
    uint32_t mask_t8x;
    const uint32_t* tile_mask;
    uint32_t* tile_mask_spare;
    uint32_t mask_words;
    const uint32_t* tile_depth;
    float rcp_w, rcp_h;
    float setup_lo;
    uint32_t rect[4];
};

#ifndef VOLYM_DEV_SWITCHES
#define VOLYM_DEV_SWITCHES 0
#endif
#define VOLYM_DF_IN_LDS(fp) (!VOLYM_DEV_SWITCHES || (fp).mc_n <= 32u)
#define VOLYM_DF_LDS_BYTES 16384

enum : uint32_t {
    CULL_CUBE_HULL = 1u << 0,
    CULL_OBJ_HULL = 1u << 1,
    CULL_AABB = 1u << 2,
    CULL_NOTHING_DENSE = 1u << 3,
    CULL_TILE_MASK = 1u << 4,
    CULL_TILE_DEPTH = 1u << 5,
};

struct FrameTables {
    float4 tf_tab[256];
    float4 lut_f[256];
    float ic_alpha[256];
    float rho[256];
};

struct Counters {
    unsigned long long n_vol, n_imp, n_steps, n_dense, n_hit;
};

struct V3 {
    float x, y, z;
};
__device__ __forceinline__ V3 v3(float x, float y, float z) { return V3{x, y, z}; }
__device__ __forceinline__ V3 operator+(V3 a, V3 b) { return v3(a.x + b.x, a.y + b.y, a.z + b.z); }
__device__ __forceinline__ V3 operator-(V3 a, V3 b) { return v3(a.x - b.x, a.y - b.y, a.z - b.z); }
__device__ __forceinline__ V3 operator*(V3 a, float s) { return v3(a.x * s, a.y * s, a.z * s); }
__device__ __forceinline__ V3 operator/(V3 a, float s) { return v3(a.x / s, a.y / s, a.z / s); }
__device__ __forceinline__ float dot_exact(V3 a, V3 b) { return (a.x * b.x + a.y * b.y) + a.z * b.z; }
__device__ __forceinline__ V3 cross(V3 a, V3 b)
{
    return v3(a.y * b.z - a.z * b.y, a.z * b.x - a.x * b.z, a.x * b.y - a.y * b.x);
}
__device__ __forceinline__ float length_exact(V3 a) { return __builtin_sqrtf(dot_exact(a, a)); }
__device__ __forceinline__ V3 normalize_exact(V3 a) { return a / length_exact(a); }
__device__ __forceinline__ float dot_fast(V3 a, V3 b)
{
    return __builtin_fmaf(a.z, b.z, __builtin_fmaf(a.y, b.y, a.x * b.x));
}

__host__ __device__ inline uint32_t brick_count(uint32_t n) { return (n + 3u) >> 2; }

template <bool BRICK>
struct GridT {
    static constexpr bool bricked = BRICK;
    const uint8_t* __restrict__ vol;
    const uint8_t* __restrict__ imp;
    int nx, ny, nz;
    uint32_t bx, bxy;
    float fnx, fny, fnz;
    float hix, hiy, hiz;
};
typedef GridT<false> Grid;

__host__ __device__ inline uint32_t layout_offset(bool bricked, uint32_t bx, uint32_t bxy, uint32_t ix, uint32_t iy, uint32_t iz)
{
    if (bricked) return (((iz >> 2) * bxy + (iy >> 2) * bx + (ix >> 2)) << 6) | ((iz & 3u) << 4) | ((iy & 3u) << 2) | (ix & 3u);
    return ix + bx * iy + bxy * iz;
}
__host__ __device__ inline uint32_t layout_bx(bool bricked, uint32_t nx) { return bricked ? brick_count(nx) : nx; }
__host__ __device__ inline uint32_t layout_bxy(bool bricked, uint32_t nx, uint32_t ny) { return bricked ? brick_count(nx) * brick_count(ny) : nx * ny; }

template <class G>
__device__ __forceinline__ void grid_init(G& g, const uint8_t* vol, const uint8_t* imp, uint32_t nx, uint32_t ny, uint32_t nz)
{
    g.vol = vol; g.imp = imp;
    g.nx = static_cast<int>(nx); g.ny = static_cast<int>(ny); g.nz = static_cast<int>(nz);
    g.bx = layout_bx(G::bricked, nx); g.bxy = layout_bxy(G::bricked, nx, ny);
    g.fnx = static_cast<float>(nx); g.fny = static_cast<float>(ny); g.fnz = static_cast<float>(nz);
    g.hix = static_cast<float>(nx - 1u); g.hiy = static_cast<float>(ny - 1u); g.hiz = static_cast<float>(nz - 1u);
}

__device__ __forceinline__ int floor_to_int(float x)
{
    int r;
    asm("v_cvt_flr_i32_f32 %0, %1" : "=v"(r) : "v"(x));
    return r;
}

__device__ __forceinline__ int clamp_texel(int i, int hi)
{
    int r;
    asm("v_med3_i32 %0, %1, 0, %2" : "=v"(r) : "v"(i), "v"(hi));
    return r;
}

__device__ __forceinline__ uint32_t mad_u24(uint32_t a, uint32_t b_uniform, uint32_t c)
{
    uint32_t r;
    asm("v_mad_u32_u24 %0, %1, %2, %3" : "=v"(r) : "v"(a), "s"(b_uniform), "v"(c));
// ... 442 lines not shown
    return __builtin_fmaf(e, r, q);
}
__device__ __forceinline__ float div_pixel(float g, float w, float r)
{
    const float q = g * r;
    return __builtin_fmaf(__builtin_fmaf(-w, q, g), r, q);
}

struct Ray {
    V3 o, d;
    float t_entry, t_exit;
    bool hit;
};

__device__ __forceinline__ void ray_slabs(Ray& r, float t1x, float t2x, float t1y, float t2y, float t1z, float t2z)
{
    const float entry = __builtin_fmaxf(__builtin_fmaxf(__builtin_fminf(t1x, t2x), __builtin_fminf(t1y, t2y)),
                                        __builtin_fminf(t1z, t2z));
    const float exit_ = __builtin_fminf(__builtin_fminf(__builtin_fmaxf(t1x, t2x), __builtin_fmaxf(t1y, t2y)),
                                        __builtin_fmaxf(t1z, t2z));
    r.t_entry = __builtin_fmaxf(entry, 0.0f);
    r.t_exit = __builtin_fmaxf(exit_, 0.0f);
    r.hit = !(r.t_exit <= r.t_entry);
}

__device__ __forceinline__ Ray make_ray_ieee(const FrameParams& fp, uint32_t gx, uint32_t gy)
{
    Ray r;
    const float scx = static_cast<float>(gx) / static_cast<float>(fp.W);
    const float scy = static_cast<float>(gy) / static_cast<float>(fp.H);
    const float ndx = scx * 2.0f - 1.0f;
    const float ndy = 1.0f - scy * 2.0f;
    float wp[4];
#pragma unroll
    for (int k = 0; k < 4; ++k)
        wp[k] = ((fp.ivp[k] * ndx + fp.ivp[4 + k] * ndy) + fp.ivp[8 + k] * 0.0f) + fp.ivp[12 + k] * 1.0f;
    r.o = v3(fp.eye[0], fp.eye[1], fp.eye[2]);
    const V3 world = v3(wp[0] / wp[3], wp[1] / wp[3], wp[2] / wp[3]);
    r.d = normalize_exact(world - r.o);
    ray_slabs(r, (0.0f - r.o.x) / r.d.x, (1.0f - r.o.x) / r.d.x, (0.0f - r.o.y) / r.d.y, (1.0f - r.o.y) / r.d.y,
              (0.0f - r.o.z) / r.d.z, (1.0f - r.o.z) / r.d.z);
    return r;
}

__device__ __forceinline__ Ray make_ray_shared(const FrameParams& fp, uint32_t gx, uint32_t gy, bool& ok)
{
    Ray r;
    const float scx = div_pixel(static_cast<float>(gx), static_cast<float>(fp.W), fp.rcp_w);
    const float scy = div_pixel(static_cast<float>(gy), static_cast<float>(fp.H), fp.rcp_h);
    const float ndx = scx * 2.0f - 1.0f;
    const float ndy = 1.0f - scy * 2.0f;
    float wp[4];
#pragma unroll
    for (int k = 0; k < 4; ++k)
        wp[k] = ((fp.ivp[k] * ndx + fp.ivp[4 + k] * ndy) + fp.ivp[8 + k] * 0.0f) + fp.ivp[12 + k] * 1.0f;
    r.o = v3(fp.eye[0], fp.eye[1], fp.eye[2]);
    const float rw = rcp_refined(wp[3]);
    const V3 a = v3(div_by(wp[0], wp[3], rw), div_by(wp[1], wp[3], rw), div_by(wp[2], wp[3], rw)) - r.o;
    const float len = length_exact(a);
    const float rl = rcp_refined(len);
    r.d = v3(div_by(a.x, len, rl), div_by(a.y, len, rl), div_by(a.z, len, rl));
    const float rx = rcp_refined(r.d.x), ry = rcp_refined(r.d.y), rz = rcp_refined(r.d.z);
    ray_slabs(r, div_by(0.0f - r.o.x, r.d.x, rx), div_by(1.0f - r.o.x, r.d.x, rx), div_by(0.0f - r.o.y, r.d.y, ry),
              div_by(1.0f - r.o.y, r.d.y, ry), div_by(0.0f - r.o.z, r.d.z, rz), div_by(1.0f - r.o.z, r.d.z, rz));
    const float lo = __builtin_fminf(__builtin_fminf(__builtin_fminf(__builtin_fabsf(wp[0]), __builtin_fabsf(wp[1])), __builtin_fabsf(wp[2])),
                                     __builtin_fminf(__builtin_fabsf(wp[3]), len));
    const float hi = __builtin_fmaxf(__builtin_fmaxf(__builtin_fmaxf(__builtin_fabsf(wp[0]), __builtin_fabsf(wp[1])), __builtin_fabsf(wp[2])),
                                     __builtin_fmaxf(__builtin_fabsf(wp[3]), len));
    const float dlo = __builtin_fminf(__builtin_fminf(__builtin_fabsf(r.d.x), __builtin_fabsf(r.d.y)), __builtin_fabsf(r.d.z));
    ok = lo > fp.setup_lo && hi < 0x1p+40f && dlo > 0x1p-30f;
    return r;
}

template <bool SHARED = true>
__device__ __forceinline__ Ray make_ray(const FrameParams& fp, uint32_t gx, uint32_t gy)
{
    if constexpr (!SHARED) return make_ray_ieee(fp, gx, gy);
    bool ok;
    const Ray r = make_ray_shared(fp, gx, gy, ok);
    if (__builtin_expect(__ballot(!ok) == 0ull, 1)) return r;
    return make_ray_ieee(fp, gx, gy);
}

}
```

volym_amd/csrc/raymarch_kernels.h:

```cpp
#pragma once

#include "raymarch_device.h"

namespace volym {

__device__ __forceinline__ uint32_t block_to_local_tile(uint32_t b, uint32_t n_local, uint32_t bands)
{
    if (bands == 0u) return b;
    const uint32_t xcd = b & 7u;
    const uint32_t i = b >> 3;
    const uint32_t chunks = 8u * bands;
    const uint32_t per_chunk = (n_local + chunks - 1u) / chunks;
    const uint32_t band = i / per_chunk;
    const uint32_t within = i - band * per_chunk;
    return (band * 8u + xcd) * per_chunk + within;
}

struct MarchCtx {
    const float4* s_tf_tab;
    const float4* s_lut;
    const float* s_ic_alpha;
    const float* s_rho;
    uint32_t flags;
    bool linear, table_mode;
// ... 446 lines not shown
                        const uint32_t end_in = (last >> 5) == word ? (last & 31u) : 31u;
                        const uint32_t m = (end_in == 31u ? 0xffffffffu : ((1u << (end_in + 1u)) - 1u)) & ~((1u << first_in) - 1u);
                        if (word < n_words) atomicOr(&s_mask[word], m);
                        bit = (word + 1u) << 5;
                    }
                }
            }
        }
    }
    const bool any_all = __syncthreads_or(all_bits ? 1 : 0) != 0;
    for (uint32_t i = threadIdx.x; i < n_words; i += 256u) {
        const uint32_t v = any_all ? 0xffffffffu : s_mask[i];
        if (v) atomicOr(&out[i], v);
    }
}

constexpr uint32_t VOLYM_TILE_DEPTH_LDS = 4096;
__global__ __launch_bounds__(256) void volym_tile_depth_kernel(const uint8_t* __restrict__ mc_max, uint32_t mc_n, uint32_t thr_byte, ClipMatrix M,
                                                               float margin, float ex, float ey, float ez, uint32_t W, uint32_t H, uint32_t t8x,
                                                               uint32_t n_t8, uint32_t* __restrict__ out)
{
    __shared__ uint32_t s_near[VOLYM_TILE_DEPTH_LDS], s_far[VOLYM_TILE_DEPTH_LDS];
    __shared__ uint32_t s_rect[4];
    if (threadIdx.x == 0u) { s_rect[0] = 0xffffffffu; s_rect[1] = 0xffffffffu; s_rect[2] = 0u; s_rect[3] = 0u; }
    __syncthreads();
    const uint32_t nbx = (mc_n + 7u) / 8u, nby = (mc_n + 7u) / 8u;
    const uint32_t bx = blockIdx.x % nbx, by = (blockIdx.x / nbx) % nby, bz = blockIdx.x / (nbx * nby);
    const uint32_t cx = bx * 8u + (threadIdx.x & 7u), cy = by * 8u + ((threadIdx.x >> 3) & 7u), cz = bz * 4u + (threadIdx.x >> 6);
    CellRect r = {0u, 0u, 0u, 0u, false, false};
    uint32_t ne = 0u, fe = 0u;
    if (cx < mc_n && cy < mc_n && cz < mc_n && mc_max[cx + mc_n * (cy + mc_n * cz)] >= thr_byte) {
        r = cell_tile_rect(M, cx, cy, cz, mc_n, margin, W, H);
        if (r.on && !r.bad) {
            float lo[3], hi[3];
            cell_box(cx, cy, cz, mc_n, margin, lo, hi);
            const float e[3] = {ex, ey, ez};
            float dn = 0.0f, df = 0.0f;
#pragma unroll
            for (int k = 0; k < 3; ++k) {
                const float a = e[k] - fminf(fmaxf(e[k], lo[k]), hi[k]);
                const float b = fmaxf(fabsf(e[k] - lo[k]), fabsf(e[k] - hi[k]));
                dn += a * a; df += b * b;
            }
            const float near = fmaxf(sqrtf(dn) * (1.0f - 2.0e-5f) - 1.0e-5f, 0.0f);
            const float far = sqrtf(df) * (1.0f + 2.0e-5f) + 1.0e-5f;
            ne = ~__float_as_uint(near); fe = __float_as_uint(far);
            atomicMin(&s_rect[0], r.tx0); atomicMin(&s_rect[1], r.ty0);
            atomicMax(&s_rect[2], r.tx1); atomicMax(&s_rect[3], r.ty1);
        }
    }
    if (__syncthreads_or(r.bad ? 1 : 0)) {
        for (uint32_t i = threadIdx.x; i < n_t8; i += 256u) { atomicMax(&out[i], 0xffffffffu); atomicMax(&out[n_t8 + i], 0x7f800000u); }
        return;
    }
    const uint32_t rx0 = s_rect[0], ry0 = s_rect[1], rx1 = s_rect[2], ry1 = s_rect[3];
    if (rx0 > rx1) return;
    const uint32_t rw = rx1 - rx0 + 1u, area = rw * (ry1 - ry0 + 1u);
    const bool lds = area <= VOLYM_TILE_DEPTH_LDS;
    if (lds) {
        for (uint32_t i = threadIdx.x; i < area; i += 256u) { s_near[i] = 0u; s_far[i] = 0u; }
        __syncthreads();
    }
    if (fe != 0u) {
        for (uint32_t ty = r.ty0; ty <= r.ty1; ++ty)
            for (uint32_t tx = r.tx0; tx <= r.tx1; ++tx) {
                if (lds) {
                    const uint32_t i = (ty - ry0) * rw + (tx - rx0);
                    atomicMax(&s_near[i], ne); atomicMax(&s_far[i], fe);
                } else {
                    const uint32_t i = ty * t8x + tx;
                    if (i < n_t8) { atomicMax(&out[i], ne); atomicMax(&out[n_t8 + i], fe); }
                }
            }
    }
    if (!lds) return;
    __syncthreads();
    for (uint32_t i = threadIdx.x; i < area; i += 256u) {
        const uint32_t f = s_far[i];
        const uint32_t t = (ry0 + i / rw) * t8x + rx0 + i % rw;
        if (f != 0u && t < n_t8) { atomicMax(&out[t], s_near[i]); atomicMax(&out[n_t8 + t], f); }
    }
}

__global__ __launch_bounds__(256) void volym_macrocell_kernel(const uint8_t* __restrict__ vol, uint8_t* __restrict__ mc_max,
                                                              uint32_t nx, uint32_t ny, uint32_t nz, uint32_t mc_n, uint32_t bricked)
{
    const uint32_t cell = blockIdx.x;
    const uint32_t cx = cell % mc_n, cy = (cell / mc_n) % mc_n, cz = cell / (mc_n * mc_n);
    auto lo = [&](uint32_t c, uint32_t n) { uint32_t v = static_cast<uint32_t>((static_cast<uint64_t>(c) * n) / mc_n); return v > 0u ? v - 1u : 0u; };
    auto hi = [&](uint32_t c, uint32_t n) { uint32_t v = static_cast<uint32_t>((static_cast<uint64_t>(c + 1u) * n + mc_n - 1u) / mc_n) + 1u; return v < n ? v : n; };
    const uint32_t x0 = lo(cx, nx), x1 = hi(cx, nx), y0 = lo(cy, ny), y1 = hi(cy, ny), z0 = lo(cz, nz), z1 = hi(cz, nz);
    const uint32_t wx = x1 - x0, wy = y1 - y0, wz = z1 - z0;
    const uint32_t total = wx * wy * wz;
    uint32_t m = 0;
    for (uint32_t i = threadIdx.x; i < total; i += 256u) {
        const uint32_t x = x0 + i % wx, y = y0 + (i / wx) % wy, z = z0 + i / (wx * wy);
        const uint32_t v = vol[layout_offset(bricked != 0u, layout_bx(bricked != 0u, nx), layout_bxy(bricked != 0u, nx, ny), x, y, z)];
        m = v > m ? v : m;
    }
    for (int s = 32; s > 0; s >>= 1) { const uint32_t o = __shfl_xor(m, s, 64); m = o > m ? o : m; }
    __shared__ uint32_t s_m[4];
    if ((threadIdx.x & 63u) == 0u) s_m[threadIdx.x >> 6] = m;
    __syncthreads();
    if (threadIdx.x == 0) {
        uint32_t r = s_m[0];
        for (int w = 1; w < 4; ++w) r = s_m[w] > r ? s_m[w] : r;
        mc_max[cell] = static_cast<uint8_t>(r);
    }
}

__global__ __launch_bounds__(256) void volym_rebrick_kernel(const uint8_t* __restrict__ linear, uint8_t* __restrict__ bricked,
                                                            uint32_t nx, uint32_t ny, uint32_t nz)
{
    const uint32_t bx = brick_count(nx), by = brick_count(ny), bz = brick_count(nz);
    const uint64_t total = static_cast<uint64_t>(bx) * by * bz * 64u;
    const uint64_t o = static_cast<uint64_t>(blockIdx.x) * 256u + threadIdx.x;
    if (o >= total) return;
    const uint32_t brick = static_cast<uint32_t>(o >> 6), in = static_cast<uint32_t>(o & 63u);
    const uint32_t x = (brick % bx) * 4u + (in & 3u), y = ((brick / bx) % by) * 4u + ((in >> 2) & 3u), z = (brick / (bx * by)) * 4u + (in >> 4);
    uint8_t v = 0;
    if (x < nx && y < ny && z < nz) v = linear[static_cast<size_t>(x) + static_cast<size_t>(nx) * (y + static_cast<size_t>(ny) * z)];
    bricked[o] = v;
}

struct LabelTable { uint8_t v[256]; };

__device__ __forceinline__ void label_chunk_origin(bool bricked, uint32_t k, uint32_t nx, uint32_t ny, uint32_t& x, uint32_t& y, uint32_t& z)
{
    if (bricked) {
        const uint32_t bx = brick_count(nx), by = brick_count(ny), brick = k >> 2;
        x = (brick % bx) * 4u; y = ((brick / bx) % by) * 4u; z = (brick / (bx * by)) * 4u + (k & 3u);
    } else {
        const uint32_t o = k * 16u, slab = nx * ny;
        z = o / slab; y = (o - z * slab) / nx; x = o - z * slab - y * nx;
    }
}

__device__ __forceinline__ uint32_t label_chunk_inside(bool bricked, uint32_t k, uint32_t nx, uint32_t ny, uint32_t nz, uint64_t n)
{
    if (!bricked) {
        const uint64_t o = static_cast<uint64_t>(k) * 16u;
        return o + 16u <= n ? 0xffffu : (1u << static_cast<uint32_t>(n - o)) - 1u;
    }
    uint32_t x, y, z;
    label_chunk_origin(true, k, nx, ny, x, y, z);
    if (z >= nz) return 0u;
    const uint32_t wx = nx - x < 4u ? nx - x : 4u, wy = ny - y < 4u ? ny - y : 4u;
    const uint32_t row = (1u << wx) - 1u;
    uint32_t m = 0;
    for (uint32_t r = 0; r < wy; ++r) m |= row << (4u * r);
    return m;
}

__global__ __launch_bounds__(256) void volym_segment_map_kernel(const uint4* __restrict__ labels, uint4* __restrict__ imp, LabelTable table,
                                                                uint32_t nx, uint32_t ny, uint32_t nz, uint32_t bricked, uint32_t n_chunks)
{
    __shared__ uint8_t s_tab[256];
    s_tab[threadIdx.x] = table.v[threadIdx.x];
    __syncthreads();
    const uint64_t n = static_cast<uint64_t>(nx) * ny * nz;
    const uint32_t stride = gridDim.x * 256u;
    auto map = [&](uint4 v, uint32_t inside) {
        uint32_t w[4] = {v.x, v.y, v.z, v.w};
#pragma unroll
        for (int j = 0; j < 4; ++j) {
            uint32_t o = 0;
// ... 133 lines not shown
```

volym_amd/csrc/raymarch_pq.h:

```cpp
#pragma once

#include <type_traits>

#include "raymarch_device.h"

namespace volym {

constexpr int PQ_WAVES = 16;
constexpr int PQ_WAVES_WIDE = 12;
constexpr uint32_t PQ_MIN_LEAP_D = 2;
constexpr int PQ_DP_DEPTH = 2;
constexpr uint32_t PQ_NO_ITEM = 0xffffffffu;
constexpr int PQ_ITEMS_LDS = 512;
constexpr int pq_qcap(int k) { return 64 + 64 * k; }
constexpr float PQ_FIX_SCALE = 268435456.0f;
constexpr float PQ_FIX_INV = 1.0f / 268435456.0f;

__device__ __forceinline__ uint32_t lane_rank_in_mask(unsigned long long mask)
{
    return __builtin_amdgcn_mbcnt_hi(static_cast<uint32_t>(mask >> 32), __builtin_amdgcn_mbcnt_lo(static_cast<uint32_t>(mask), 0u));
}

typedef float f32x2 __attribute__((ext_vector_type(2)));

enum : uint32_t { TILE_MARCH = 0, TILE_HIT_TEST = 1, TILE_FILL_EMPTY = 2, TILE_FILL_MISS = 3 };

struct HullEdge { float a, b, c; bool valid; };
__device__ __forceinline__ HullEdge load_hull_edge(const FrameParams& fp, uint32_t lane)
{
    const uint32_t h = lane >> 5, e = (lane >> 2) & 7u;
    HullEdge r;
    r.a = fp.hull[h][e][0]; r.b = fp.hull[h][e][1]; r.c = fp.hull[h][e][2]; r.valid = fp.hull[h][e][3] > 0.5f;
    return r;
}
__device__ __forceinline__ uint32_t classify_tile(const FrameParams& fp, const HullEdge& edge, uint32_t lane, float x0, float y0, float extent = 7.0f,
                                                   bool masked_out = false)
{
    const uint32_t k = lane & 3u;
    const float cx = (k & 1u) ? x0 + extent : x0, cy = (k & 2u) ? y0 + extent : y0;
    const float a = edge.a, b = edge.b, c = edge.c;
    const bool valid = edge.valid;
    const float v = __builtin_fmaf(a, cx, __builtin_fmaf(b, cy, c));
    const float margin = 1.5f;
    const unsigned long long mo = __ballot(valid && v < -margin);
    const unsigned long long mi = __ballot(!valid || v > margin);
    auto outside = [&](uint32_t bits) { return ((bits & (bits >> 1) & (bits >> 2) & (bits >> 3)) & 0x11111111u) != 0u; };
    const bool cube_ok = (fp.cull & CULL_CUBE_HULL) != 0u, obj_ok = (fp.cull & CULL_OBJ_HULL) != 0u;
    const bool out_cube = cube_ok && outside(static_cast<uint32_t>(mo));
    const bool in_cube = cube_ok && static_cast<uint32_t>(mi) == 0xffffffffu;
    const bool out_obj = masked_out || (fp.cull & CULL_NOTHING_DENSE) != 0u || (obj_ok && outside(static_cast<uint32_t>(mo >> 32)));
    if (out_cube) return TILE_FILL_MISS;
    if (out_obj) return in_cube ? TILE_FILL_EMPTY : TILE_HIT_TEST;
    return TILE_MARCH;
}
__device__ __forceinline__ bool tile_mask_bit(const FrameParams& fp, uint32_t t8x, uint32_t t8y)
{
    const uint32_t bit = t8y * fp.mask_t8x + t8x;
    return ((fp.tile_mask[bit >> 5] >> (bit & 31u)) & 1u) != 0u;
}
template <bool TABLE, bool COUNT, bool TRACE = false, int KSPEC = 1, bool IMP = true, bool BRICK = false, bool IR = false, int WAVES = PQ_WAVES, int CJ = 0, bool LB = false>
__global__ __launch_bounds__(WAVES * 64) void volym_raymarch_pq_kernel(
    const uint8_t* __restrict__ vol, const uint8_t* __restrict__ imp, const FrameTables* __restrict__ tables,
    const uint8_t* __restrict__ df4, const uint2* __restrict__ order, uint32_t n_items, uint16_t* __restrict__ cost,
    uint32_t* __restrict__ out_shard, uint32_t* __restrict__ out_raster, float4* __restrict__ out_f32,
    Counters* __restrict__ counters, uint4* __restrict__ trace, const FrameParams fp)
{
    constexpr int K = TABLE ? KSPEC : 2;
    constexpr int PQ_QCAP = pq_qcap(K);
    static_assert(K <= 4, "the shading queue of K > 4 does not fit the LDS");
    static_assert(CJ == 0 || IR, "look-ahead jobs belong to the importance-rendering instantiation");
    unsigned long long trace_t0 = 0;
    uint32_t trace_iters = 0, trace_flushes = 0, trace_tiles = 0, trace_marched = 0, trace_lanes = 0, trace_accepted = 0, trace_dp_iters = 0;
    unsigned long long tm_leap = 0, tm_samp = 0, tm_flush = 0, tm_mark = 0;
#define PQ_TICK() (TRACE ? __builtin_amdgcn_s_memtime() : 0ull)
    if (TRACE) trace_t0 = __builtin_amdgcn_s_memrealtime();

    __shared__ float4 s_tf_tab[256];
    __shared__ float4 s_lut[TABLE ? 1 : 256];
    __shared__ float s_ic_alpha[256];
    __shared__ float s_rho[256];
    __shared__ __attribute__((aligned(16))) uint8_t s_df[VOLYM_DF_LDS_BYTES];
    constexpr int THREADS = WAVES * 64;
    __shared__ float4 s_q[WAVES][PQ_QCAP];
    __shared__ uint32_t s_qm[WAVES][PQ_QCAP];
    __shared__ float s_qr[TABLE ? 1 : WAVES][TABLE ? 1 : PQ_QCAP];
    __shared__ uint32_t s_acc[WAVES][3][64];
    __shared__ float4 s_hh[WAVES][64];
    __shared__ uint8_t s_mail[(IMP || IR) ? WAVES : 1][(IMP || IR) ? 256 : 1];
    uint8_t (*const s_cres)[(IMP || IR) ? 256 : 1] = s_mail;
    constexpr uint32_t CJ_LPR = CJ == 2 ? 1u : 8u;
    constexpr uint32_t CJ_RPS = 64u / CJ_LPR;
    constexpr uint32_t CJ_CAP = CJ == 2 ? 64u : 32u;
    static_assert(!LB || (TABLE && BRICK && !IMP && !IR && !COUNT && K == 4), "LDS brick staging: bricked layout, common instantiation");
    constexpr uint32_t LB_SLOTS = 8u;
    __shared__ uint32_t s_lb[LB ? WAVES : 1][LB ? LB_SLOTS * 16u : 1u];
    constexpr int ITEMS_LDS = LB ? PQ_ITEMS_LDS / 4 : CJ == 2 ? PQ_ITEMS_LDS / 2 : PQ_ITEMS_LDS;
    __shared__ float4 s_cj[CJ ? 2 * CJ_CAP : 1];
    __shared__ uint32_t s_cj_flag[CJ ? CJ_CAP : 1];
    __shared__ uint32_t s_cj_ctl[4];
    __shared__ uint32_t s_next_ticket;
    __shared__ uint2 s_items[ITEMS_LDS];

    static_assert(!(IMP && IR), "IR specialises the IMP = false paths");
    const uint32_t flags = IMP ? fp.flags : IR ? ((fp.flags & ~F_IMP_COLORING) | F_OPACITY | F_IMP_RENDERING)
                                               : ((fp.flags & ~(F_IMP_COLORING | F_IMP_RENDERING | F_CONE)) | F_OPACITY);
    const bool linear = (flags & F_LINEAR) != 0u;
    const bool gauss = (flags & F_GAUSSIAN) != 0u;
    const bool imp_coloring = IMP && (flags & F_IMP_COLORING) != 0u;
    const bool imp_rendering = (IMP || IR) && (flags & F_IMP_RENDERING) != 0u;
    const bool need_imp = imp_coloring || imp_rendering;

    if (fp.tile_mask_spare)
        for (uint32_t wrd = blockIdx.x * (WAVES * 64u) + threadIdx.x; wrd < fp.mask_words; wrd += gridDim.x * (WAVES * 64u)) fp.tile_mask_spare[wrd] = 0u;
    if (VOLYM_DEV_SWITCHES && (fp.dev & 16u)) return;
    uint32_t* const wg_time = reinterpret_cast<uint32_t*>(cost + ((n_items + 1u) & ~1u));
    if (cost && threadIdx.x == 0u) wg_time[gridDim.x * WAVES + blockIdx.x] = static_cast<uint32_t>(__builtin_amdgcn_s_memrealtime());
    {
        const uint32_t i = threadIdx.x;
        if (i == 0u) s_next_ticket = 0u;
        if (CJ) {
            for (uint32_t k = i; k < CJ_CAP; k += THREADS) s_cj_flag[k] = 0u;
            if (i == 0u) { s_cj_ctl[0] = 0u; s_cj_ctl[1] = 0u; s_cj_ctl[2] = WAVES; }
        }
        for (uint32_t k = i; k < static_cast<uint32_t>(ITEMS_LDS); k += THREADS) {
            const size_t gi = blockIdx.x + static_cast<size_t>(gridDim.x) * k;
            if (gi < n_items) s_items[k] = order[gi];
        }
        if (i < 256u) {
            s_tf_tab[i] = tables->tf_tab[i];
            s_rho[i] = tables->rho[i];
            s_ic_alpha[i] = tables->ic_alpha[i];
            if (!TABLE) s_lut[i] = tables->lut_f[i];
        }
        {
            const uint32_t n16 = VOLYM_DF_IN_LDS(fp) ? (fp.mc_n * fp.mc_n * fp.mc_n / 2u + 15u) / 16u : 0u;
            const uint4* src = reinterpret_cast<const uint4*>(df4);
            uint4* dst = reinterpret_cast<uint4*>(s_df);
            if (!(VOLYM_DEV_SWITCHES && (fp.dev & 8u)))
                for (uint32_t k = i; k < n16; k += THREADS) dst[k] = src[k];
        }
    }
    __syncthreads();
    if (VOLYM_DEV_SWITCHES && (fp.dev & 4u)) return;

    const uint32_t lane = threadIdx.x & 63u;
    const uint32_t wave = __builtin_amdgcn_readfirstlane(threadIdx.x >> 6);

    GridT<BRICK> g;
    grid_init(g, vol, imp, fp.nx, fp.ny, fp.nz);

    float4* const q4 = s_q[wave];
    uint32_t* const qm = s_qm[wave];
    float* const qr = s_qr[TABLE ? 0 : wave];
    uint32_t* const acc_r = s_acc[wave][0];
    uint32_t* const acc_g = s_acc[wave][1];
    uint32_t* const acc_b = s_acc[wave][2];
    float4* const hh = s_hh[wave];
    uint8_t* const mail = s_mail[(IMP || IR) ? wave : 0];

    uint32_t lb_tag = 0xffffffffu, lb_next = 0u;
    uint32_t n_vol = 0, n_imp = 0, n_steps = 0, n_dense = 0, n_hit = 0;
    const float base = fp.base_step, min_step = fp.min_step, thr = fp.thr;
    const float mcf = static_cast<float>(fp.mc_n), inv_mc = 1.0f / mcf;

    const uint32_t n_mine = n_items > blockIdx.x ? (n_items - blockIdx.x + gridDim.x - 1) / gridDim.x : 0u;
    auto grab = [&]() __attribute__((always_inline)) -> uint32_t {
        uint32_t ticket = 0;
        if (lane == 0) ticket = atomicAdd(&s_next_ticket, 1u);
        return __builtin_amdgcn_readfirstlane(ticket);
    };
    const bool culling = !COUNT && fp.cull != 0u;
    const HullEdge hull_edge = load_hull_edge(fp, lane);

    uint32_t cj_count = 0;
    uint32_t la_rounds = 0;
    auto cj_serve = [&]() __attribute__((always_inline)) -> bool {
// ... 190 lines not shown
        }
        const uint32_t raw0 = raw_p & ~0x30000000u;
        const bool is_super = (raw0 >> 30) == 1u;
        uint32_t n_sub = 1;
        if (is_super) {
            const uint32_t lt = raw0 & 0x3fffffffu;
            const uint32_t tx16 = tx, ty16 = ty;
            bool masked16 = false;
            if (culling && (fp.cull & CULL_TILE_MASK))
                masked16 = !(tile_mask_bit(fp, tx16 * 2u, ty16 * 2u) || tile_mask_bit(fp, tx16 * 2u + 1u, ty16 * 2u) ||
                             tile_mask_bit(fp, tx16 * 2u, ty16 * 2u + 1u) || tile_mask_bit(fp, tx16 * 2u + 1u, ty16 * 2u + 1u));
            const uint32_t cls = culling ? classify_tile(fp, hull_edge, lane, static_cast<float>(tx16 * 16u), static_cast<float>(ty16 * 16u), 15.0f, masked16) : TILE_MARCH;
            if (cls >= TILE_FILL_EMPTY) {
                const uint32_t packed = cls == TILE_FILL_MISS ? 0xff000000u : 0u;
                if (flags & F_RASTER) {
                    const uint32_t gx4 = tx16 * 16u + (lane & 3u) * 4u, gy4 = ty16 * 16u + (lane >> 2);
                    if (gy4 < fp.H && (fp.W & 3u) == 0u && (reinterpret_cast<uintptr_t>(out_raster) & 15u) == 0u && gx4 < fp.W && !(flags & F_WRITE_F32)) {
                        *reinterpret_cast<uint4*>(out_raster + static_cast<size_t>(gy4) * fp.W + gx4) = make_uint4(packed, packed, packed, packed);
                    } else if (gy4 < fp.H) {
                        for (uint32_t i = 0; i < 4u; ++i)
                            if (gx4 + i < fp.W) {
                                out_raster[static_cast<size_t>(gy4) * fp.W + gx4 + i] = packed;
                                if (flags & F_WRITE_F32) out_f32[static_cast<size_t>(gy4) * fp.W + gx4 + i] = make_float4(0.0f, 0.0f, 0.0f, cls == TILE_FILL_MISS ? 1.0f : 0.0f);
                            }
                    }
                } else {
                    for (uint32_t i = 0; i < 4u; ++i) {
                        const uint32_t sl = lane * 4u + i, sub4 = sl >> 6, in = sl & 63u;
                        const uint32_t gxx = tx16 * 16u + ((sub4 & 1u) << 3) + (in & 7u), gyy = ty16 * 16u + ((sub4 >> 1) << 3) + (in >> 3);
                        out_shard[static_cast<size_t>(lt) * 256u + sl] = (gxx < fp.W && gyy < fp.H) ? packed : 0u;
                    }
                }
                if (cost && lane == 0) cost[list_pos] = 0;
                continue;
            }
            n_sub = 4;
        }
      for (uint32_t sub_iter = 0; sub_iter < n_sub; ++sub_iter) {
        const uint32_t raw = is_super ? ((raw0 & 0x3fffffffu) * 4u + sub_iter) : raw0;
        const bool is_quarter = (raw >> 31) != 0u;
        const bool dp = is_quarter && !COUNT;
        const uint32_t item = is_quarter ? ((raw & 0x7fffffffu) >> 2) : raw;
        const uint32_t quarter = raw & 3u;
        if (is_quarter && !dp && quarter != 0u) continue;
        const uint32_t local_tile = item >> 2, sub = item & 3u;
        const uint32_t px_in_sub = dp ? (((quarter & 1u) << 2) + ((lane >> 2) & 3u)) : (lane & 7u);
        const uint32_t py_in_sub = dp ? (((quarter >> 1) << 2) + (lane >> 4)) : (lane >> 3);
        const uint32_t sub_lane = py_in_sub * 8u + px_in_sub;
        const uint32_t own = dp ? (lane & ~3u) : lane;
        const uint32_t gx = tx * 16u + ((sub & 1u) << 3) + px_in_sub;
        const uint32_t gy = ty * 16u + ((sub >> 1) << 3) + py_in_sub;
        const bool in_frame = gx < fp.W && gy < fp.H;

        if (TRACE) { trace_tiles++; tm_mark = PQ_TICK(); }
        uint32_t tile_iters = 0, tile_flushes = 0, tile_trips = 0;
        const uint32_t cj_at_start = cj_count, la_at_start = la_rounds;
        uint32_t trace_ray_iters = 0;
        uint32_t tclass = TILE_MARCH;
        if (culling && !dp) {
            const bool masked8 = (fp.cull & CULL_TILE_MASK) != 0u && !tile_mask_bit(fp, tx * 2u + (sub & 1u), ty * 2u + (sub >> 1));
            tclass = classify_tile(fp, hull_edge, lane, static_cast<float>(tx * 16u + ((sub & 1u) << 3)), static_cast<float>(ty * 16u + ((sub >> 1) << 3)), 7.0f, masked8);
            if (tclass >= TILE_FILL_EMPTY) {
                const uint32_t packed = tclass == TILE_FILL_MISS ? 0xff000000u : 0u;
                if (flags & F_RASTER) {
                    if (in_frame) {
                        const size_t o = static_cast<size_t>(gy) * fp.W + gx;
                        out_raster[o] = packed;
                        if (flags & F_WRITE_F32) out_f32[o] = make_float4(0.0f, 0.0f, 0.0f, tclass == TILE_FILL_MISS ? 1.0f : 0.0f);
                    }
                } else {
                    out_shard[static_cast<size_t>(local_tile) * 256u + sub * 64u + sub_lane] = in_frame ? packed : 0u;
                }
                continue;
            }
        }
        if (TRACE) trace_marched++;

        acc_r[lane] = 0u; acc_g[lane] = 0u; acc_b[lane] = 0u;
        uint32_t q_head = 0, q_count = 0;

        Ray ray;
        ray.o = v3(0.0f, 0.0f, 0.0f); ray.d = v3(0.0f, 0.0f, 0.0f); ray.t_entry = 0.0f; ray.t_exit = 0.0f;
        ray.hit = false;
        if (in_frame) ray = make_ray<TABLE && !IMP && !IR>(fp, gx, gy);
        {
            const V3 hvec = ray_half_vector(ray.d);
            hh[lane] = make_float4(hvec.x, hvec.y, hvec.z, 0.0f);
        }
        bool active = in_frame && ray.hit;
        if (COUNT && active) n_hit++;
        float t = active ? ray.t_entry : 0.0f, cur = base, acc_a = active ? 0.0f : 1.0f;
        bool last_dense = false;
        if (culling && tclass == TILE_HIT_TEST) active = false;
        float t_end = ray.t_exit;
        if (culling && (fp.cull & CULL_AABB) && active) {
            const float rx = __builtin_amdgcn_rcpf(ray.d.x), ry = __builtin_amdgcn_rcpf(ray.d.y), rz = __builtin_amdgcn_rcpf(ray.d.z);
            const float ax0 = (fp.aabb_lo[0] - ray.o.x) * rx, ax1 = (fp.aabb_hi[0] - ray.o.x) * rx;
            const float ay0 = (fp.aabb_lo[1] - ray.o.y) * ry, ay1 = (fp.aabb_hi[1] - ray.o.y) * ry;
            const float az0 = (fp.aabb_lo[2] - ray.o.z) * rz, az1 = (fp.aabb_hi[2] - ray.o.z) * rz;
            float tn = __builtin_fmaxf(__builtin_fmaxf(__builtin_fminf(ax0, ax1), __builtin_fminf(ay0, ay1)), __builtin_fminf(az0, az1));
            float tf = __builtin_fminf(__builtin_fminf(__builtin_fmaxf(ax0, ax1), __builtin_fmaxf(ay0, ay1)), __builtin_fmaxf(az0, az1));
            tn = tn - 2.0e-5f * __builtin_fabsf(tn) - 1.0e-6f;
            tf = tf + 2.0e-5f * __builtin_fabsf(tf) + 1.0e-6f;
            if (fp.cull & CULL_TILE_DEPTH) {
                const auto* td = (const __attribute__((address_space(4))) uint32_t*)fp.tile_depth;
                const uint32_t t8 = (ty * 2u + (sub >> 1)) * fp.mask_t8x + tx * 2u + (sub & 1u);
                tn = __builtin_fmaxf(tn, __uint_as_float(~td[t8]));
                tf = __builtin_fminf(tf, __uint_as_float(td[32u * fp.mask_words + t8]));
            }
            const bool outside_static = (ray.d.x == 0.0f && (ray.o.x < fp.aabb_lo[0] || ray.o.x > fp.aabb_hi[0])) ||
                                        (ray.d.y == 0.0f && (ray.o.y < fp.aabb_lo[1] || ray.o.y > fp.aabb_hi[1])) ||
                                        (ray.d.z == 0.0f && (ray.o.z < fp.aabb_lo[2] || ray.o.z > fp.aabb_hi[2]));
            if (outside_static || !(tn <= tf)) {
                active = false;
            } else {
                t_end = __builtin_fminf(t_end, tf);
                const float t_first = __builtin_fminf(tn, t_end);
                replay_saturated(t, t_first, base);
            }
        }
        const float idx_ = __builtin_amdgcn_rcpf(ray.d.x), idy_ = __builtin_amdgcn_rcpf(ray.d.y), idz_ = __builtin_amdgcn_rcpf(ray.d.z);
        const float nox = -ray.o.x * idx_, noy = -ray.o.y * idy_, noz = -ray.o.z * idz_;

        auto flush = [&](uint32_t n) __attribute__((always_inline)) {
            unsigned long long fl0 = 0;
            tile_flushes++;
            if (TRACE) { trace_flushes++; fl0 = PQ_TICK(); }
            __builtin_amdgcn_fence(__ATOMIC_SEQ_CST, "wavefront");
            __builtin_amdgcn_wave_barrier();
            if (lane < n && !(VOLYM_DEV_SWITCHES && (fp.dev & 1u))) {
                const uint32_t e0 = q_head + lane, e = min(e0, e0 - PQ_QCAP);
                const float4 rec = q4[e];
                const V3 pos = v3(rec.x, rec.y, rec.z);
                const float w = rec.w;
                const uint32_t meta = qm[e];
                const uint32_t owner = meta & 63u, b = (meta >> 8) & 255u, ib = (meta >> 16) & 255u;
                V3 color;
                if (imp_coloring) {
                    const float im = s_rho[ib];
                    color = v3(__builtin_fminf(im * 1.5f, 1.0f), (1.0f - im) * 1.2f, 0.2f);
                } else if (TABLE) {
                    const float4 ca = s_tf_tab[b];
                    color = v3(ca.x, ca.y, ca.z);
                } else {
                    const float4 ca = sample_tf(s_lut, fp.tf_n, qr[e]);
                    color = v3(ca.x, ca.y, ca.z);
                }
                V3 grad;
                const float o = 0.01f;
                if (TABLE) {
                    const int ix = texel_nearest(pos.x, g.fnx, g.hix), iy = texel_nearest(pos.y, g.fny, g.hiy),
                              iz = texel_nearest(pos.z, g.fnz, g.hiz);
                    const f32x2 pm = {o, -o};
                    const f32x2 uxs = (pos.x + pm) * g.fnx, uys = (pos.y + pm) * g.fny, uzs = (pos.z + pm) * g.fnz;
                    const int ixp = clamp_texel(floor_to_int(uxs.x), static_cast<int>(g.hix)), ixm = clamp_texel(floor_to_int(uxs.y), static_cast<int>(g.hix));
                    const int iyp = clamp_texel(floor_to_int(uys.x), static_cast<int>(g.hiy)), iym = clamp_texel(floor_to_int(uys.y), static_cast<int>(g.hiy));
                    const int izp = clamp_texel(floor_to_int(uzs.x), static_cast<int>(g.hiz)), izm = clamp_texel(floor_to_int(uzs.y), static_cast<int>(g.hiz));
                    const int bxp = vol[voxel_offset(g, ixp, iy, iz)], bxm = vol[voxel_offset(g, ixm, iy, iz)];
                    const int byp = vol[voxel_offset(g, ix, iyp, iz)], bym = vol[voxel_offset(g, ix, iym, iz)];
                    const int bzp = vol[voxel_offset(g, ix, iy, izp)], bzm = vol[voxel_offset(g, ix, iy, izm)];
                    grad = v3(static_cast<float>(bxp - bxm), static_cast<float>(byp - bym), static_cast<float>(bzp - bzm));
                } else {
                    grad = v3(sample_density(g, s_rho, linear, v3(pos.x + o, pos.y, pos.z)) -
                                  sample_density(g, s_rho, linear, v3(pos.x - o, pos.y, pos.z)),
                              sample_density(g, s_rho, linear, v3(pos.x, pos.y + o, pos.z)) -
                                  sample_density(g, s_rho, linear, v3(pos.x, pos.y - o, pos.z)),
                              sample_density(g, s_rho, linear, v3(pos.x, pos.y, pos.z + o)) -
                                  sample_density(g, s_rho, linear, v3(pos.x, pos.y, pos.z - o)));
                }
                const float4 hv = hh[owner];
                const V3 shaded = blinn_phong_h(color, grad, v3(hv.x, hv.y, hv.z));
                atomicAdd(&acc_r[owner], static_cast<uint32_t>(__builtin_fmaf(shaded.x * w, PQ_FIX_SCALE, 0.5f)));
                atomicAdd(&acc_g[owner], static_cast<uint32_t>(__builtin_fmaf(shaded.y * w, PQ_FIX_SCALE, 0.5f)));
                atomicAdd(&acc_b[owner], static_cast<uint32_t>(__builtin_fmaf(shaded.z * w, PQ_FIX_SCALE, 0.5f)));
            }
            q_head += n;
            if (q_head >= PQ_QCAP) q_head -= PQ_QCAP;
            q_count -= n;
            __builtin_amdgcn_fence(__ATOMIC_SEQ_CST, "wavefront");
            __builtin_amdgcn_wave_barrier();
            if (TRACE) tm_flush += PQ_TICK() - fl0;
        };

        auto append = [&](bool emit, V3 p, float w, uint32_t meta, float rho) __attribute__((always_inline)) {
            if (VOLYM_DEV_SWITCHES && (fp.dev & 128u)) return;
            const unsigned long long mask = __ballot(emit);
            if (mask == 0ull) return;
            if (emit) {
                const uint32_t e0 = q_head + q_count + lane_rank_in_mask(mask), e = min(e0, e0 - PQ_QCAP);
                q4[e] = make_float4(p.x, p.y, p.z, w); qm[e] = meta;
                if (!TABLE) qr[e] = rho;
            }
            q_count += static_cast<uint32_t>(__popcll(mask));
            if (!TABLE && q_count >= 64u) flush(64u);
        };
        auto drain = [&]() __attribute__((always_inline)) { while (q_count >= 64u) flush(64u); };

        if (VOLYM_DEV_SWITCHES && (fp.dev & 256u)) active = false;
        if (TRACE) tm_mark = PQ_TICK();
        bool leap_ok = true;
        auto leap_phase = [&]() __attribute__((always_inline)) {
            active = active && t < t_end && acc_a < 0.95f;
// ... 589 lines not shown
```

volym_amd/demo.py:

```python
import ctypes as C

import numpy as np

from . import _lib, scene, synth


class GpuContext:

    def __init__(self, width, height, device_id=-1):
        self.width, self.height = int(width), int(height)
        self._h = C.c_void_p()
        rc = _lib.lib().volym_create(C.byref(self._h), self.width, self.height, int(device_id))
        if rc != _lib.OK:
            raise _lib.VolymError(rc, (_lib.lib().volym_last_error(None) or b"").decode())

    @classmethod
    def borrow(cls, handle, width, height):
        self = cls.__new__(cls)
        self.width, self.height = int(width), int(height)
        self._h = handle
        self._borrowed = True
        return self

    @property
# ... 72 lines not shown

    def update(self, camera_uniforms, parameter_uniforms):
        self._ck(_lib.lib().volym_update(self.handle, C.byref(camera_uniforms), C.byref(parameter_uniforms)))

    def compute_pass(self):
        self._ck(_lib.lib().volym_compute_pass(self.handle))

    def sync(self):
        self._ck(_lib.lib().volym_sync(self.handle))

    def throttle(self, max_in_flight=3):
        self._ck(_lib.lib().volym_throttle(self.handle, int(max_in_flight)))

    def settle(self):
        self._ck(_lib.lib().volym_settle(self.handle))

    def blit(self, out_w, out_h, target_ptr=None):
        self._blit_size = (int(out_h), int(out_w))
        self._ck(_lib.lib().volym_blit(self.handle, C.c_void_p(target_ptr), int(out_w), int(out_h)))

    def read_blit(self):
        h, w = self._blit_size
        out = np.empty((h, w, 4), np.uint8)
        self._ck(_lib.lib().volym_read_blit(self.handle, scene._u8p(out)))
        return out

    def read_rgba8(self):
        out = np.empty((self.height, self.width, 4), np.uint8)
        self._ck(_lib.lib().volym_read_rgba8(self.handle, scene._u8p(out)))
        return out

    def read_rgba32f(self):
        out = np.empty((self.height, self.width, 4), np.float32)
        self._ck(_lib.lib().volym_read_rgba32f(self.handle, scene._f32p(out)))
        return out

    def local_tiles(self):
        return int(_lib.lib().volym_local_tiles(self.handle))

    def shard_bytes(self):
        return int(_lib.lib().volym_shard_bytes(self.handle))

    def shard_device_ptr(self):
        return _lib.lib().volym_shard_device_ptr(self.handle)

    def frame_device_ptr(self):
        return _lib.lib().volym_frame_device_ptr(self.handle)

    def read_shard(self):
        out = np.empty(self.shard_bytes(), np.uint8)
        self._ck(_lib.lib().volym_read_shard(self.handle, scene._u8p(out)))
        return out

    def assemble(self, gathered_device_ptr):
        self._ck(_lib.lib().volym_assemble(self.handle, C.c_void_p(gathered_device_ptr)))

    def packed_shard_bytes(self, tiles):
        return int(_lib.lib().volym_packed_shard_bytes(self.handle, int(tiles)))

    def pack_shard(self, packed_device_ptr, capacity_bytes):
        self._ck(_lib.lib().volym_pack_shard(self.handle, C.c_void_p(packed_device_ptr), int(capacity_bytes)))

    def packed_tiles(self):
        used, over = C.c_uint32(0), C.c_uint32(0)
        self._ck(_lib.lib().volym_packed_tiles(self.handle, C.byref(used), C.byref(over)))
        return int(used.value), int(over.value)

    def assemble_packed(self, gathered_device_ptr, stride_bytes):
        self._ck(_lib.lib().volym_assemble_packed(self.handle, C.c_void_p(gathered_device_ptr), int(stride_bytes)))

    def assemble_host(self, gathered):
        g = np.ascontiguousarray(gathered, np.uint8).ravel()
        self._ck(_lib.lib().volym_assemble_host(self.handle, scene._u8p(g)))

    def stats_pass(self):
        s = _lib.Stats()
        self._ck(_lib.lib().volym_stats_pass(self.handle, C.byref(s)))
        return s.as_dict()

    def selftest_ray_setup(self):
        out = (C.c_ulonglong * 3)()
        self._ck(_lib.lib().volym_selftest_ray_setup(self.handle, out))
        return int(out[0]), int(out[1]), int(out[2])

    def time_batch(self, n):
        ms = C.c_float(0.0)
        self._ck(_lib.lib().volym_time_batch(self.handle, int(n), C.byref(ms)))
        return float(ms.value)

    def time_passes(self, n):
        ms = np.zeros(int(n), np.float32)
        self._ck(_lib.lib().volym_time_passes(self.handle, int(n), scene._f32p(ms)))
        return ms


class ComputeDemo:

    @classmethod
    def init(cls, ctx, state, **kw):
        raise NotImplementedError

    def update_gpu_state(self, ctx, state):
        raise NotImplementedError

    def compute_pass(self, ctx):
        raise NotImplementedError


class Simple(ComputeDemo):

    def __init__(self, dims):
        self.dims = dims

    @classmethod
    def init(cls, ctx, state, volume_raw=None, labels_raw=None, segments=None, dims=(256, 256, 256),
             filter=_lib.FILTER_NEAREST, transfer_function=None):
        if volume_raw is None:
            volume_raw, labels_raw = synth.synth_teapot()
            segments = synth.TEAPOT_SEGMENTS
        if labels_raw is None:
            labels_raw = np.zeros(0, np.uint8)
        segments = scene.load_segments(segments if segments is not None else [])
        volume = scene.prepare_volume(volume_raw, dims, flip_y=True)
        ctx.set_volume(volume, dims, filter)
        importances = scene.prepare_volume(scene.map_segments_to_importance(labels_raw, segments), dims, flip_y=True)
        ctx.set_importances(importances, dims)
        tf = transfer_function if transfer_function is not None else scene.TransferFunction.default()
        ctx.set_transfer_function(tf.bake_rgba8())
        self = cls(dims)
        self.update_gpu_state(ctx, state)
        return self

    def update_gpu_state(self, ctx, state):
        ctx.update(state.camera_uniforms(), state.parameter_uniforms())

    def compute_pass(self, ctx):
        ctx.compute_pass()

    def set_labels(self, ctx, labels_raw):
        labels_raw = np.ascontiguousarray(labels_raw, np.uint8).ravel()
        ctx.set_labels(scene.prepare_volume(labels_raw, self.dims, flip_y=True), self.dims)
        self._labels_raw = labels_raw
        self._labels_on_device = True

    def set_segments(self, ctx, segments):
        segments = scene.load_segments(segments)
        table = scene.segment_table(segments)
        padded = self._labels_raw.size < self.dims[0] * self.dims[1] * self.dims[2]
        if padded and table[0] != 0:
            importances = scene.map_segments_to_importance(self._labels_raw, segments)
            ctx.set_importances(scene.prepare_volume(importances, self.dims, flip_y=True), self.dims)
            self._labels_on_device = False
            return
        if not self._labels_on_device:
            self.set_labels(ctx, self._labels_raw)
        ctx.set_segment_importances(table)
```

Measured before the change: 83120.

## Cache per-view ray setup in a precomputed buffer read by the march kernel

Adds a ray-setup kernel that runs when the view changes. For each 8x8 tile it stores ray direction, clipped entry and exit t, the half vector and active/hit ballots. A new RC instantiation of the PQ march kernel loads these values instead of recomputing make_ray and the AABB/tile-depth clipping per pass. This swaps per-pass ALU work for extra global memory reads and buffer allocation, and it only covers the common no-importance opacity path. The shard change now marks the hull dirty so the cached rays are rebuilt.

```diff
diff --git a/include/volym_hip.h b/include/volym_hip.h
--- a/include/volym_hip.h
+++ b/include/volym_hip.h
@@ -115,6 +115,9 @@
 int volym_time_batch(volym_ctx* ctx, uint32_t n, float* ms_total);
 int volym_selftest_ray_setup(volym_ctx* ctx, unsigned long long out[3]);
 
+enum { VOLYM_VIEW_TILE_MASK = 1, VOLYM_VIEW_TILE_DEPTH = 2, VOLYM_VIEW_RAY_SETUP = 4, VOLYM_VIEW_RAY_SETUP_READ = 8 };
+int volym_view_structures(volym_ctx* ctx, uint32_t* out);
+
 #ifdef __cplusplus
 }
 #endif
diff --git a/volym_amd/_lib.py b/volym_amd/_lib.py
--- a/volym_amd/_lib.py
+++ b/volym_amd/_lib.py
@@ -142,6 +142,7 @@
     "volym_time_passes": (C.c_int, [_ctx, C.c_uint32, _f32p]),
     "volym_time_batch": (C.c_int, [_ctx, C.c_uint32, _f32p]),
     "volym_selftest_ray_setup": (C.c_int, [_ctx, C.POINTER(C.c_ulonglong)]),
+    "volym_view_structures": (C.c_int, [_ctx, C.POINTER(C.c_uint32)]),
     "volym_camera_default_with_aspect_and_pos": (None, [C.POINTER(CCamera), C.c_float, _f32p]),
     "volym_camera_orbit": (None, [C.POINTER(CCamera), C.c_float, C.c_float, C.c_float]),
     "volym_camera_view_matrix": (None, [C.POINTER(CCamera), _f32p]),
diff --git a/volym_amd/csrc/context.hpp b/volym_amd/csrc/context.hpp
--- a/volym_amd/csrc/context.hpp
+++ b/volym_amd/csrc/context.hpp
@@ -78,6 +78,9 @@
     float mask_clip[16] = {};
     float mask_margin = 0.0f;
     uint32_t* d_tile_depth = nullptr;
+    float4* d_ray_cache = nullptr;
+    bool last_read_ray_setup = false;
+    uint4* d_ray_state = nullptr;
     int* d_aabb = nullptr;
 
     uint32_t* d_shard_own = nullptr;
@@ -150,6 +153,7 @@
     uint32_t tile_mask_words = 0;
     bool tile_mask = true;
     bool tile_depth = true;
+    bool ray_cache = true;
     bool mask_eager = false;
 
     uint32_t* bound_shard = nullptr;
diff --git a/volym_amd/csrc/raymarch.hip b/volym_amd/csrc/raymarch.hip
--- a/volym_amd/csrc/raymarch.hip
+++ b/volym_amd/csrc/raymarch.hip
@@ -17,6 +17,9 @@
 
 namespace volym {
 extern template __global__ void volym_raymarch_pq_kernel<true, false, false, 4, false, false, false, PQ_WAVES, 0, false>(
+    const uint8_t* __restrict__, const uint8_t* __restrict__, const FrameTables* __restrict__, const uint8_t* __restrict__, const uint2* __restrict__, uint32_t,
+    uint16_t* __restrict__, uint32_t* __restrict__, uint32_t* __restrict__, float4* __restrict__, Counters* __restrict__, uint4* __restrict__, const FrameParams);
+extern template __global__ void volym_raymarch_pq_kernel<true, false, false, 4, false, false, false, PQ_WAVES, 0, false, true>(
     const uint8_t* __restrict__, const uint8_t* __restrict__, const FrameTables* __restrict__, const uint8_t* __restrict__, const uint2* __restrict__, uint32_t,
     uint16_t* __restrict__, uint32_t* __restrict__, uint32_t* __restrict__, float4* __restrict__, Counters* __restrict__, uint4* __restrict__, const FrameParams);
 }
@@ -699,7 +702,7 @@
     (void)hipFree(s.d_tables); (void)hipFree(s.d_df);
     (void)hipFree(s.d_shard_own); (void)hipFree(s.d_frame_own); (void)hipFree(s.d_f32); (void)hipFree(s.d_blit);
     (void)hipFree(s.d_gather_tmp); (void)hipFree(s.d_pack_counters); (void)hipFree(s.d_counters); (void)hipFree(s.d_aabb); (void)hipFree(s.d_tile_mask);
-    (void)hipFree(s.d_tile_depth);
+    (void)hipFree(s.d_tile_depth); (void)hipFree(s.d_ray_cache); (void)hipFree(s.d_ray_state);
     (void)hipFree(s.d_list[0]); (void)hipFree(s.d_list[1]); (void)hipFree(s.d_cost);
     (void)hipFree(s.d_pool_sync); (void)hipFree(s.d_pool_dbg);
     if (s.h_list_pinned) (void)hipHostFree(s.h_list_pinned);
@@ -918,6 +921,10 @@
         c->tile_depth = value != 0;
         for (int i = 0; i < c->n_slots(); ++i) c->slots[i]->hull_dirty = true;
         return rebuild_lists(c);
+    case 124:
+        c->ray_cache = value != 0;
+        for (int i = 0; i < c->n_slots(); ++i) c->slots[i]->hull_dirty = true;
+        return rebuild_lists(c);
     case 117:
         c->tile_mask = value != 0;
         c->mask_eager = value == 2;
@@ -941,6 +948,7 @@
     if (rc != VOLYM_OK) return rc;
     c->rank = rank; c->world = world;
     recompute_shard(c);
+    for (int i = 0; i < c->n_slots(); ++i) c->slots[i]->hull_dirty = true;
     return rebuild_lists(c);
 }
 
@@ -1141,6 +1149,23 @@
 
 }
 
+static bool ray_cache_wanted(const volym_ctx* c, const FrameSlot& s)
+{
+    const uint32_t f = s.fp.flags;
+    return c->ray_cache && c->kernel_variant == 2 && !(f & (F_LINEAR | F_GAUSSIAN | F_IMP_COLORING | F_IMP_RENDERING)) && (f & F_OPACITY);
+}
+
+static bool ensure_ray_cache(volym_ctx* c, FrameSlot& s)
+{
+    if (s.d_ray_cache && s.d_ray_state) return true;
+    hipStreamCaptureStatus cs = hipStreamCaptureStatusNone;
+    if (hipStreamIsCapturing(s.stream, &cs) != hipSuccess || cs != hipStreamCaptureStatusNone) return false;
+    const size_t n_t8 = 32u * static_cast<size_t>(c->tile_mask_words);
+    if (!s.d_ray_cache && hipMalloc(&s.d_ray_cache, 128u * n_t8 * sizeof(float4)) != hipSuccess) { s.d_ray_cache = nullptr; (void)hipGetLastError(); return false; }
+    if (!s.d_ray_state && hipMalloc(&s.d_ray_state, n_t8 * sizeof(uint4)) != hipSuccess) { s.d_ray_state = nullptr; (void)hipGetLastError(); return false; }
+    return true;
+}
+
 static int ensure_frame_resources(volym_ctx* c, FrameSlot& s)
 {
     if (s.df_thr_byte != s.thr_byte_cull) {
@@ -1154,6 +1179,8 @@
         compute_culling(c, s);
         s.fp.tile_mask = nullptr;
         s.fp.tile_depth = nullptr;
+        s.fp.ray_cache = nullptr;
+        s.fp.ray_state = nullptr;
         s.fp.mask_words = c->tile_mask_words;
         s.fp.tile_mask_spare = s.d_tile_mask ? s.d_tile_mask + static_cast<size_t>(s.mask_cur ^ 1) * c->tile_mask_words : nullptr;
         s.mask_pending = s.mask_wanted;
@@ -1185,6 +1212,15 @@
             HIPCHK(c, hipGetLastError());
             s.fp.tile_depth = s.d_tile_depth;
             s.fp.cull |= CULL_TILE_DEPTH;
+            if (ray_cache_wanted(c, s) && s.d_ray_cache && s.d_ray_state) {
+                const uint32_t t8_rows = c->tiles_y * 2u, n_t8_frame = c->tiles_x * 2u * t8_rows;
+                hipLaunchKernelGGL(volym_ray_setup_kernel, dim3((n_t8_frame + 3u) / 4u), dim3(256), 0, s.stream, s.fp, t8_rows, c->rank, c->world,
+                                   s.d_ray_cache, s.d_ray_state);
+                HIPCHK(c, hipGetLastError());
+                s.fp.ray_cache = s.d_ray_cache;
+                s.fp.ray_state = s.d_ray_state;
+                s.fp.cull |= CULL_RAY_CACHE;
+            }
         }
         s.fp.tile_mask_spare = s.d_tile_mask + static_cast<size_t>(s.mask_cur ^ 1) * c->tile_mask_words;
         s.mask_pending = false;
@@ -1256,6 +1292,7 @@
     } else {
         s.thr_byte_cull = tb;
     }
+    if (c->tile_mask_words && ray_cache_wanted(c, s)) (void)ensure_ray_cache(c, s);
     if (view_changed) {
         s.view_serial.fetch_add(1, std::memory_order_relaxed);
         s.hull_dirty = true;
@@ -1302,6 +1339,7 @@
     int rc = ensure_frame_resources(c, s);
     if (rc != VOLYM_OK) return rc;
     FrameParams fp = s.fp;
+    s.last_read_ray_setup = false;
     fp.rank = c->rank; fp.world = c->world; fp.n_local = c->n_local;
     fp.mc_n = c->mc_n;
     fp.xcd_bands = c->xcd_bands;
@@ -1356,6 +1394,12 @@
 #else
 #define VOLYM_PQ_LAUNCH_W(T, KS, I, B, R) VOLYM_PQ_LAUNCH(T, KS, I, B, R, PQ_WAVES)
 #endif
+        const bool ray_cache = (fp.cull & CULL_RAY_CACHE) != 0u && !COUNT && !TRACE;
+        s.last_read_ray_setup = ray_cache && table && no_imp && !(VOLYM_DEV_SWITCHES && c->bricked && c->lds_bricks);
+#define VOLYM_PQ_LAUNCH_RC(B)                                                                                                     \
+    hipLaunchKernelGGL((volym_raymarch_pq_kernel<true, false, false, 4, false, B, false, PQ_WAVES, 0, false, true>), dim3(pgrid), dim3(PQ_WAVES * 64), 0, \
+                       s.stream, c->d_vol, c->d_imp, s.d_tables, s.d_df, reinterpret_cast<const uint2*>(s.d_list[s.cur]), n_items, cost_out, d_shard, \
+                       d_frame, s.d_f32, cnt, trace, fp)
         const bool cone_jobs = ir && (fp.flags & F_CONE) != 0u && !TRACE;
         const bool straight_jobs = VOLYM_DEV_SWITCHES && ir && !(fp.flags & F_CONE) && !TRACE && c->straight_jobs;
         (void)straight_jobs;
@@ -1366,7 +1410,8 @@
                                    c->d_imp, s.d_tables, s.d_df, reinterpret_cast<const uint2*>(s.d_list[s.cur]), n_items, cost_out, d_shard, d_frame, s.d_f32, cnt, trace, fp);
             else
 #endif
-            if (table && no_imp) VOLYM_PQ_LAUNCH(true, 4, false, true, false, PQ_WAVES);
+            if (table && no_imp && ray_cache) VOLYM_PQ_LAUNCH_RC(true);
+            else if (table && no_imp) VOLYM_PQ_LAUNCH(true, 4, false, true, false, PQ_WAVES);
             else if (table && ir && cone_jobs) VOLYM_PQ_LAUNCH_J(true, 4, false, true, true, PQ_WAVES, 1);
 #if VOLYM_DEV_SWITCHES
             else if (table && ir && straight_jobs) VOLYM_PQ_LAUNCH_J(true, 4, false, true, true, PQ_WAVES, 2);
@@ -1375,7 +1420,8 @@
             else if (table) VOLYM_PQ_LAUNCH_W(true, 4, true, true, false);
             else VOLYM_PQ_LAUNCH_W(false, 1, true, true, false);
         } else {
-            if (table && no_imp) VOLYM_PQ_LAUNCH(true, 4, false, false, false, PQ_WAVES);
+            if (table && no_imp && ray_cache) VOLYM_PQ_LAUNCH_RC(false);
+            else if (table && no_imp) VOLYM_PQ_LAUNCH(true, 4, false, false, false, PQ_WAVES);
             else if (table && ir && cone_jobs) VOLYM_PQ_LAUNCH_J(true, 4, false, false, true, PQ_WAVES, 1);
 #if VOLYM_DEV_SWITCHES
             else if (table && ir && straight_jobs) VOLYM_PQ_LAUNCH_J(true, 4, false, false, true, PQ_WAVES, 2);
@@ -1387,6 +1433,7 @@
 #undef VOLYM_PQ_LAUNCH_W
 #undef VOLYM_PQ_LAUNCH
 #undef VOLYM_PQ_LAUNCH_J
+#undef VOLYM_PQ_LAUNCH_RC
         HIPCHK(c, hipGetLastError());
         if (capture) {
             HIPCHK(c, hipEventRecord(s.ev_march, s.stream));
@@ -1698,6 +1745,15 @@
     return VOLYM_OK;
 }
 
+int volym_view_structures(volym_ctx* c, uint32_t* out)
+{
+    if (!c || !out) return VOLYM_E_INVALID;
+    const FrameSlot& s = *c->slots[c->last];
+    *out = ((s.fp.cull & CULL_TILE_MASK) ? VOLYM_VIEW_TILE_MASK : 0u) | ((s.fp.cull & CULL_TILE_DEPTH) ? VOLYM_VIEW_TILE_DEPTH : 0u) |
+           ((s.fp.cull & CULL_RAY_CACHE) ? VOLYM_VIEW_RAY_SETUP : 0u) | (s.last_read_ray_setup ? VOLYM_VIEW_RAY_SETUP_READ : 0u);
+    return VOLYM_OK;
+}
+
 int volym_selftest_ray_setup(volym_ctx* c, unsigned long long out[3])
 {
     if (!c || !out) return VOLYM_E_INVALID;
diff --git a/volym_amd/csrc/raymarch_common.hip b/volym_amd/csrc/raymarch_common.hip
--- a/volym_amd/csrc/raymarch_common.hip
+++ b/volym_amd/csrc/raymarch_common.hip
@@ -7,5 +7,8 @@
 template __global__ void volym_raymarch_pq_kernel<true, false, false, 4, false, false, false, PQ_WAVES, 0, false>(
     const uint8_t* __restrict__, const uint8_t* __restrict__, const FrameTables* __restrict__, const uint8_t* __restrict__, const uint2* __restrict__, uint32_t,
     uint16_t* __restrict__, uint32_t* __restrict__, uint32_t* __restrict__, float4* __restrict__, Counters* __restrict__, uint4* __restrict__, const FrameParams);
+template __global__ void volym_raymarch_pq_kernel<true, false, false, 4, false, false, false, PQ_WAVES, 0, false, true>(
+    const uint8_t* __restrict__, const uint8_t* __restrict__, const FrameTables* __restrict__, const uint8_t* __restrict__, const uint2* __restrict__, uint32_t,
+    uint16_t* __restrict__, uint32_t* __restrict__, uint32_t* __restrict__, float4* __restrict__, Counters* __restrict__, uint4* __restrict__, const FrameParams);
 
 }
diff --git a/volym_amd/csrc/raymarch_device.h b/volym_amd/csrc/raymarch_device.h
--- a/volym_amd/csrc/raymarch_device.h
+++ b/volym_amd/csrc/raymarch_device.h
@@ -46,6 +46,8 @@
     uint32_t* tile_mask_spare;
     uint32_t mask_words;
     const uint32_t* tile_depth;
+    const float4* ray_cache;
+    const uint4* ray_state;
     float rcp_w, rcp_h;
     float setup_lo;
     uint32_t rect[4];
@@ -64,6 +66,7 @@
     CULL_NOTHING_DENSE = 1u << 3,
     CULL_TILE_MASK = 1u << 4,
     CULL_TILE_DEPTH = 1u << 5,
+    CULL_RAY_CACHE = 1u << 6,
 };
 
 struct FrameTables {
@@ -672,4 +675,31 @@
     return make_ray_ieee(fp, gx, gy);
 }
 
-}
+__device__ __forceinline__ void clip_ray_entry(const FrameParams& fp, const Ray& ray, uint32_t t8, float base, float& t, float& t_end, bool& active)
+{
+    const float rx = __builtin_amdgcn_rcpf(ray.d.x), ry = __builtin_amdgcn_rcpf(ray.d.y), rz = __builtin_amdgcn_rcpf(ray.d.z);
+    const float ax0 = (fp.aabb_lo[0] - ray.o.x) * rx, ax1 = (fp.aabb_hi[0] - ray.o.x) * rx;
+    const float ay0 = (fp.aabb_lo[1] - ray.o.y) * ry, ay1 = (fp.aabb_hi[1] - ray.o.y) * ry;
+    const float az0 = (fp.aabb_lo[2] - ray.o.z) * rz, az1 = (fp.aabb_hi[2] - ray.o.z) * rz;
+    float tn = __builtin_fmaxf(__builtin_fmaxf(__builtin_fminf(ax0, ax1), __builtin_fminf(ay0, ay1)), __builtin_fminf(az0, az1));
+    float tf = __builtin_fminf(__builtin_fminf(__builtin_fmaxf(ax0, ax1), __builtin_fmaxf(ay0, ay1)), __builtin_fmaxf(az0, az1));
+    tn = tn - 2.0e-5f * __builtin_fabsf(tn) - 1.0e-6f;
+    tf = tf + 2.0e-5f * __builtin_fabsf(tf) + 1.0e-6f;
+    if (fp.cull & CULL_TILE_DEPTH) {
+        const auto* td = (const __attribute__((address_space(4))) uint32_t*)fp.tile_depth;
+        tn = __builtin_fmaxf(tn, __uint_as_float(~td[t8]));
+        tf = __builtin_fminf(tf, __uint_as_float(td[32u * fp.mask_words + t8]));
+    }
+    const bool outside_static = (ray.d.x == 0.0f && (ray.o.x < fp.aabb_lo[0] || ray.o.x > fp.aabb_hi[0])) ||
+                                (ray.d.y == 0.0f && (ray.o.y < fp.aabb_lo[1] || ray.o.y > fp.aabb_hi[1])) ||
+                                (ray.d.z == 0.0f && (ray.o.z < fp.aabb_lo[2] || ray.o.z > fp.aabb_hi[2]));
+    if (outside_static || !(tn <= tf)) {
+        active = false;
+    } else {
+        t_end = __builtin_fminf(t_end, tf);
+        const float t_first = __builtin_fminf(tn, t_end);
+        replay_saturated(t, t_first, base);
+    }
+}
+
+}
diff --git a/volym_amd/csrc/raymarch_kernels.h b/volym_amd/csrc/raymarch_kernels.h
--- a/volym_amd/csrc/raymarch_kernels.h
+++ b/volym_amd/csrc/raymarch_kernels.h
@@ -552,6 +552,36 @@
     }
 }
 
+__global__ __launch_bounds__(256) void volym_ray_setup_kernel(const FrameParams fp, uint32_t t8_rows, uint32_t rank, uint32_t world,
+                                                              float4* __restrict__ rays, uint4* __restrict__ state)
+{
+    const uint32_t lane = threadIdx.x & 63u;
+    const uint32_t t8 = __builtin_amdgcn_readfirstlane(blockIdx.x * 4u + (threadIdx.x >> 6));
+    if (t8 >= fp.mask_t8x * t8_rows) return;
+    const uint32_t t8y = t8 / fp.mask_t8x, t8x = t8 - t8y * fp.mask_t8x;
+    if (((t8y >> 1) * (fp.mask_t8x >> 1) + (t8x >> 1)) % world != rank) return;
+    const uint32_t gx = t8x * 8u + (lane & 7u), gy = t8y * 8u + (lane >> 3);
+    const bool in_frame = gx < fp.W && gy < fp.H;
+    const float base = fp.base_step;
+    Ray ray;
+    ray.o = v3(0.0f, 0.0f, 0.0f); ray.d = v3(0.0f, 0.0f, 0.0f); ray.t_entry = 0.0f; ray.t_exit = 0.0f;
+    ray.hit = false;
+    if (in_frame) ray = make_ray(fp, gx, gy);
+    const V3 hvec = ray_half_vector(ray.d);
+    bool active = in_frame && ray.hit;
+    const bool hit = active;
+    float t = active ? ray.t_entry : 0.0f, t_end = ray.t_exit;
+    if ((fp.cull & CULL_AABB) && active) clip_ray_entry(fp, ray, t8, base, t, t_end, active);
+    const unsigned long long act = __ballot(active), hits = __ballot(hit);
+    if (lane == 0u)
+        state[t8] = make_uint4(static_cast<uint32_t>(act), static_cast<uint32_t>(act >> 32), static_cast<uint32_t>(hits), static_cast<uint32_t>(hits >> 32));
+    if ((fp.tile_mask[t8 >> 5] >> (t8 & 31u)) & 1u) {
+        float4* const r = rays + static_cast<size_t>(t8) * 128u;
+        r[lane] = make_float4(ray.d.x, ray.d.y, ray.d.z, t);
+        r[64u + lane] = make_float4(t_end, hvec.x, hvec.y, hvec.z);
+    }
+}
+
 __global__ __launch_bounds__(256) void volym_macrocell_kernel(const uint8_t* __restrict__ vol, uint8_t* __restrict__ mc_max,
                                                               uint32_t nx, uint32_t ny, uint32_t nz, uint32_t mc_n, uint32_t bricked)
 {
diff --git a/volym_amd/csrc/raymarch_pq.h b/volym_amd/csrc/raymarch_pq.h
--- a/volym_amd/csrc/raymarch_pq.h
+++ b/volym_amd/csrc/raymarch_pq.h
@@ -58,7 +58,8 @@
     const uint32_t bit = t8y * fp.mask_t8x + t8x;
     return ((fp.tile_mask[bit >> 5] >> (bit & 31u)) & 1u) != 0u;
 }
-template <bool TABLE, bool COUNT, bool TRACE = false, int KSPEC = 1, bool IMP = true, bool BRICK = false, bool IR = false, int WAVES = PQ_WAVES, int CJ = 0, bool LB = false>
+template <bool TABLE, bool COUNT, bool TRACE = false, int KSPEC = 1, bool IMP = true, bool BRICK = false, bool IR = false, int WAVES = PQ_WAVES, int CJ = 0, bool LB = false,
+          bool RC = false>
 __global__ __launch_bounds__(WAVES * 64) void volym_raymarch_pq_kernel(
     const uint8_t* __restrict__ vol, const uint8_t* __restrict__ imp, const FrameTables* __restrict__ tables,
     const uint8_t* __restrict__ df4, const uint2* __restrict__ order, uint32_t n_items, uint16_t* __restrict__ cost,
@@ -92,6 +93,7 @@
     constexpr uint32_t CJ_RPS = 64u / CJ_LPR;
     constexpr uint32_t CJ_CAP = CJ == 2 ? 64u : 32u;
     static_assert(!LB || (TABLE && BRICK && !IMP && !IR && !COUNT && K == 4), "LDS brick staging: bricked layout, common instantiation");
+    static_assert(!RC || (TABLE && !IMP && !IR && !COUNT && !TRACE && !LB), "the per-view ray set-up: common instantiations only");
     constexpr uint32_t LB_SLOTS = 8u;
     __shared__ uint32_t s_lb[LB ? WAVES : 1][LB ? LB_SLOTS * 16u : 1u];
     constexpr int ITEMS_LDS = LB ? PQ_ITEMS_LDS / 4 : CJ == 2 ? PQ_ITEMS_LDS / 2 : PQ_ITEMS_LDS;
@@ -448,42 +450,43 @@
         Ray ray;
         ray.o = v3(0.0f, 0.0f, 0.0f); ray.d = v3(0.0f, 0.0f, 0.0f); ray.t_entry = 0.0f; ray.t_exit = 0.0f;
         ray.hit = false;
+        bool active;
+        float t, cur = base, acc_a, t_end;
+        bool last_dense = false;
+        if constexpr (RC) {
+            const uint32_t t8x = tx * 2u + (sub & 1u), t8y = ty * 2u + (sub >> 1), t8 = t8y * fp.mask_t8x + t8x;
+            const auto* rs = (const __attribute__((address_space(4))) uint32_t*)fp.ray_state + t8 * 4u;
+            const uint32_t a0 = rs[0], a1 = rs[1], h0 = rs[2], h1 = rs[3];
+            const uint32_t sh = sub_lane & 31u;
+            active = (((sub_lane < 32u ? a0 : a1) >> sh) & 1u) != 0u;
+            const bool hit = (((sub_lane < 32u ? h0 : h1) >> sh) & 1u) != 0u;
+            float4 e0 = make_float4(0.0f, 0.0f, 0.0f, 0.0f), e1 = e0;
+            if (tile_mask_bit(fp, t8x, t8y)) {
+                const float4* rc = fp.ray_cache + static_cast<size_t>(t8) * 128u;
+                e0 = rc[sub_lane];
+                e1 = rc[64u + sub_lane];
+            }
+            ray.o = v3(fp.eye[0], fp.eye[1], fp.eye[2]);
+            ray.d = v3(e0.x, e0.y, e0.z);
+            ray.hit = hit;
+            t = e0.w;
+            t_end = e1.x;
+            hh[lane] = make_float4(e1.y, e1.z, e1.w, 0.0f);
+            acc_a = hit ? 0.0f : 1.0f;
+            if (culling && tclass == TILE_HIT_TEST) active = false;
+        } else {
         if (in_frame) ray = make_ray<TABLE && !IMP && !IR>(fp, gx, gy);
         {
             const V3 hvec = ray_half_vector(ray.d);
             hh[lane] = make_float4(hvec.x, hvec.y, hvec.z, 0.0f);
         }
-        bool active = in_frame && ray.hit;
+        active = in_frame && ray.hit;
         if (COUNT && active) n_hit++;
-        float t = active ? ray.t_entry : 0.0f, cur = base, acc_a = active ? 0.0f : 1.0f;
-        bool last_dense = false;
+        t = active ? ray.t_entry : 0.0f; acc_a = active ? 0.0f : 1.0f;
         if (culling && tclass == TILE_HIT_TEST) active = false;
-        float t_end = ray.t_exit;
-        if (culling && (fp.cull & CULL_AABB) && active) {
-            const float rx = __builtin_amdgcn_rcpf(ray.d.x), ry = __builtin_amdgcn_rcpf(ray.d.y), rz = __builtin_amdgcn_rcpf(ray.d.z);
-            const float ax0 = (fp.aabb_lo[0] - ray.o.x) * rx, ax1 = (fp.aabb_hi[0] - ray.o.x) * rx;
-            const float ay0 = (fp.aabb_lo[1] - ray.o.y) * ry, ay1 = (fp.aabb_hi[1] - ray.o.y) * ry;
-            const float az0 = (fp.aabb_lo[2] - ray.o.z) * rz, az1 = (fp.aabb_hi[2] - ray.o.z) * rz;
-            float tn = __builtin_fmaxf(__builtin_fmaxf(__builtin_fminf(ax0, ax1), __builtin_fminf(ay0, ay1)), __builtin_fminf(az0, az1));
-            float tf = __builtin_fminf(__builtin_fminf(__builtin_fmaxf(ax0, ax1), __builtin_fmaxf(ay0, ay1)), __builtin_fmaxf(az0, az1));
-            tn = tn - 2.0e-5f * __builtin_fabsf(tn) - 1.0e-6f;
-            tf = tf + 2.0e-5f * __builtin_fabsf(tf) + 1.0e-6f;
-            if (fp.cull & CULL_TILE_DEPTH) {
-                const auto* td = (const __attribute__((address_space(4))) uint32_t*)fp.tile_depth;
-                const uint32_t t8 = (ty * 2u + (sub >> 1)) * fp.mask_t8x + tx * 2u + (sub & 1u);
-                tn = __builtin_fmaxf(tn, __uint_as_float(~td[t8]));
-                tf = __builtin_fminf(tf, __uint_as_float(td[32u * fp.mask_words + t8]));
-            }
-            const bool outside_static = (ray.d.x == 0.0f && (ray.o.x < fp.aabb_lo[0] || ray.o.x > fp.aabb_hi[0])) ||
-                                        (ray.d.y == 0.0f && (ray.o.y < fp.aabb_lo[1] || ray.o.y > fp.aabb_hi[1])) ||
-                                        (ray.d.z == 0.0f && (ray.o.z < fp.aabb_lo[2] || ray.o.z > fp.aabb_hi[2]));
-            if (outside_static || !(tn <= tf)) {
-                active = false;
-            } else {
-                t_end = __builtin_fminf(t_end, tf);
-                const float t_first = __builtin_fminf(tn, t_end);
-                replay_saturated(t, t_first, base);
-            }
+        t_end = ray.t_exit;
+        if (culling && (fp.cull & CULL_AABB) && active)
+            clip_ray_entry(fp, ray, (ty * 2u + (sub >> 1)) * fp.mask_t8x + tx * 2u + (sub & 1u), base, t, t_end, active);
         }
         const float idx_ = __builtin_amdgcn_rcpf(ray.d.x), idy_ = __builtin_amdgcn_rcpf(ray.d.y), idz_ = __builtin_amdgcn_rcpf(ray.d.z);
         const float nox = -ray.o.x * idx_, noy = -ray.o.y * idy_, noz = -ray.o.z * idz_;
diff --git a/volym_amd/demo.py b/volym_amd/demo.py
--- a/volym_amd/demo.py
+++ b/volym_amd/demo.py
@@ -178,6 +178,11 @@
         out = (C.c_ulonglong * 3)()
         self._ck(_lib.lib().volym_selftest_ray_setup(self.handle, out))
         return int(out[0]), int(out[1]), int(out[2])
+
+    def view_structures(self):
+        out = C.c_uint32(0)
+        self._ck(_lib.lib().volym_view_structures(self.handle, C.byref(out)))
+        return int(out.value)
 
     def time_batch(self, n):
         ms = C.c_float(0.0)
```

New measurement: 84900 (median of 6 runs). 1.02x the previous value.
